# Annusha/LIReC

Measured on AMD Instinct MI355X. Metric: clips/sec fwd+bwd at 16 tracks×2048-d, higher is better.
Workload: dtype f32 in/out, bf16x3 split-precision MFMA, f32 accumulate

## Files before the change

include/lirec_hip.h:

```cpp
#ifndef LIREC_HIP_H
#define LIREC_HIP_H

#include <stdint.h>

#ifdef __cplusplus
extern "C" {
#endif

typedef void* lirec_stream_t;
typedef void* lirec_ctx_t;

#define LIREC_VERSION 124
#define LIREC_MAX_SEG 4

enum {
  LIREC_OK = 0,
  LIREC_EINVAL = 10001,
  LIREC_EWORKSPACE = 10002
};

enum { LIREC_SITE_H1_INTS = 0, LIREC_SITE_H1_CTX = 1, LIREC_SITE_E_INTS = 2,
       LIREC_SITE_E_CTX = 3, LIREC_SITE_GATE = 4,
       LIREC_SITE_TRACK_SAMPLE = 5 };

// ... 66 lines not shown
  const float* W2[LIREC_MAX_SEG];
  const float* H1;
  const float* dZ2; int64_t lddz2;
  float* dW1[LIREC_MAX_SEG]; float* db1[LIREC_MAX_SEG];
  float* dW2[LIREC_MAX_SEG]; float* db2[LIREC_MAX_SEG];
  void* workspace; int64_t workspace_bytes;
  const float* mask; const float* Hbar; const float* fscale;
  const int32_t* rowmap; const int32_t* cstart; const int32_t* count;
  const float* wts;
  int32_t in_off[LIREC_MAX_SEG], in_dim[LIREC_MAX_SEG], out_dim[LIREC_MAX_SEG];
  int32_t rows, nseg, J, parts;
  int32_t R, clamp_zero;
  lirec_rowsel sel;
  lirec_dropout drop;
  int32_t x_bf16, reserved2_;
  void* planes; int64_t planes_bytes;
  const void* hbits;
  const struct lirec_pieces_s* pieces;
  int32_t x_q32, reserved3_;
  const struct lirec_fused_adam_s* adam;
} lirec_embed_bwd_args;
typedef struct lirec_fused_adam_s {
  float* p; const float* g; float* m; float* v;
  void* wq; int64_t wq_first;
  int64_t n, n_params;
  int32_t step; float lr, beta1, beta2, eps, weight_decay, grad_scale;
  const int64_t* step_dev;
} lirec_fused_adam;
int lirec_embed_bwd(const lirec_embed_bwd_args* a, lirec_stream_t stream);
int lirec_embed_bwd2(const lirec_embed_bwd_args* a, const lirec_embed_bwd_args* b, lirec_stream_t stream);
typedef struct {
  const lirec_embed_bwd_args* heads[2];
  int32_t nh, out_bf16;
  const float* W1[2][LIREC_MAX_SEG];
  void* dX; int64_t ldx;
  int32_t n, rp1, D, reserved_;
} lirec_embed_dx_args;
int lirec_embed_dx(const lirec_embed_dx_args* a, lirec_stream_t stream);
int lirec_embed_dw1_indexed(const lirec_embed_bwd_args* const* heads, int32_t nh, const lirec_pieces* pieces,
                            float* const* P, float* const* S, lirec_stream_t stream);
typedef struct {
  const lirec_embed_bwd_args* heads[2];
  int32_t nh, reserved_;
  const float* S[2];
  const float* W1[2][LIREC_MAX_SEG];
  const lirec_pieces* pieces;
  float* dClip; int64_t ld_clip;
  float* dTrack; int64_t ld_track;
} lirec_embed_dx_indexed_args;
int lirec_embed_dx_indexed(const lirec_embed_dx_indexed_args* a, lirec_stream_t stream);
int64_t lirec_workspace_bytes(int32_t rows, int32_t nseg, int32_t J);
int64_t lirec_planes_bytes(int32_t rows, int32_t dsum, int32_t J, int32_t x_mode);

int lirec_pool_fwd(const float* Z2, int64_t ldz, const float* mask, int32_t n, int32_t R, int32_t W,
                   int32_t clamp_zero, float* Tn, int64_t ldtn, float* E, int64_t lde,
                   const lirec_dropout* drop, lirec_stream_t stream);
int lirec_pool_bwd(const float* dP, int64_t lddp, const float* mask, int32_t n, int32_t R, int32_t W,
                   int32_t clamp_zero, float* dZ2, int64_t lddz, lirec_stream_t stream);

int lirec_gate_fwd(const float* EE, int64_t ldee, const float* Wg, const float* bg, int32_t n, int32_t K,
                   int32_t N, float* G, int64_t ldg, const lirec_dropout* drop, lirec_stream_t stream);
int lirec_gate_bwd(const float* dZg, int64_t lddzg, const float* EE, int64_t ldee, const float* Wg,
                   int32_t n, int32_t K, int32_t N, int32_t split,
                   const float* Tn, int64_t ldtn, float* dWg, float* dbg, float* dEE, int64_t lddee,
                   int32_t acc_first, const lirec_dropout* drop, int32_t site_ctx, int32_t site_ints,
                   lirec_stream_t stream);
int lirec_gate_bwd_parts(const float* dZg, int64_t lddzg, const float* EE, int64_t ldee, const float* Wg,
                         int32_t n, int32_t K, int32_t N, int32_t split,
                         const float* Tn, int64_t ldtn, float* dWg, float* dbg, float* dEE, int64_t lddee,
                         int32_t acc_first, const lirec_dropout* drop, int32_t site_ctx, int32_t site_ints,
                         int32_t parts, lirec_stream_t stream);

int64_t lirec_gate_ws_bytes(int32_t n, int32_t K, int32_t N);
int lirec_gate_fwd_ws(const float* EE, int64_t ldee, const float* Wg, const float* bg, int32_t n, int32_t K,
                      int32_t N, float* G, int64_t ldg, const lirec_dropout* drop, void* ws, int64_t ws_bytes,
                      int32_t weights_staged, lirec_stream_t stream);
int lirec_gate_stage_weights(const float* Wg, int32_t n, int32_t K, int32_t N, void* ws, int64_t ws_bytes, lirec_stream_t stream);
int lirec_gate_bwd_ws(const float* dZg, int64_t lddzg, const float* EE, int64_t ldee, const float* Wg,
                      int32_t n, int32_t K, int32_t N, int32_t split,
                      const float* Tn, int64_t ldtn, float* dWg, float* dbg, float* dEE, int64_t lddee,
                      int32_t acc_first, const lirec_dropout* drop, int32_t site_ctx, int32_t site_ints,
                      int32_t parts, void* ws, int64_t ws_bytes, int32_t rows_staged, lirec_stream_t stream);

int lirec_linear_fwd(const float* A, int64_t lda, const float* W, const float* b, int32_t n, int32_t K,
                     int32_t N, float* Y, int64_t ldy, lirec_stream_t stream);
int lirec_linear_bwd(const float* dY, int64_t lddy, const float* A, int64_t lda, const float* W,
                     int32_t n, int32_t K, int32_t N, float* dW, float* db,
                     float* dA, int64_t ldda, int32_t mode, const float* act, int64_t ldact,
                     int32_t accumulate, const lirec_dropout* drop, lirec_stream_t stream);

typedef struct {
  const float* A; int64_t lda; const float* W; const float* b; float* Y; int64_t ldy;
  int32_t n, K, N, reserved_;
} lirec_linear_fwd_args;
int lirec_linear_fwd_group(const lirec_linear_fwd_args* v, int32_t count, lirec_stream_t stream);
typedef struct {
  const float* dY; int64_t lddy; const float* A; int64_t lda; const float* W;
  float* dW; float* db; float* dA; int64_t ldda; const float* act; int64_t ldact;
  int32_t n, K, N, mode, accumulate;
  int32_t parts;
  lirec_dropout drop;
} lirec_linear_bwd_args;
int lirec_linear_bwd_group(const lirec_linear_bwd_args* v, int32_t count, lirec_stream_t stream);

typedef struct {
  float* ints; int64_t ld_ints;
  const float* rels; int64_t ld_rels;
  const float* mem;
  const float* w;
  const int32_t* y;
  const int32_t* r;
  const int32_t* g;
  const int32_t* sel;
  float* d_ints; int64_t ld_dints;
  float* d_rels; int64_t ld_drels;
  float* loss;
  float* partial;
  int32_t* sel_out;
  int32_t B, T, C, NR;
  float margin, lymbda;
  int32_t max_neg, tr_correct, mask_inplace, rels_mean_valid;
  int32_t loader_types;
  int32_t sample;
  uint64_t sample_seed;
  const uint64_t* sample_seed_dev;
  float* probs_out;
  int32_t* arrive;
  float batch_divisor, rels_divisor;
  const float* divisors_dev;
  int32_t y_stride, reserved_;
} lirec_margin_loss_args;
int lirec_margin_loss(const lirec_margin_loss_args* a, lirec_stream_t stream);

int lirec_heads_loss_fwd_bwd(const lirec_linear_fwd_args* heads, const lirec_linear_bwd_args* back, int32_t n_heads,
                             const lirec_margin_loss_args* loss, lirec_stream_t stream);

int lirec_ce_loss(const float* ints, int64_t ld_ints, const float* rels, int64_t ld_rels,
                  const int32_t* y, const int32_t* r, const float* class_w,
                  int32_t B, int32_t C, int32_t NR, float* d_ints, int64_t ld_dints,
                  float* d_rels, int64_t ld_drels, float* loss, float* partial,
                  float den_ints, float den_rels, const float* dens_dev, lirec_stream_t stream);

int lirec_adam_step(float* p, const float* g, float* m, float* v, int64_t n, int32_t step,
                    float lr, float beta1, float beta2, float eps, float weight_decay,
                    float grad_scale, const int64_t* step_dev, lirec_stream_t stream);
int lirec_adam_step_counted(float* p, const float* g, float* m, float* v, int64_t n,
                            float lr, float beta1, float beta2, float eps, float weight_decay,
                            float grad_scale, int64_t* count_dev, int32_t* ticket, int32_t advance, lirec_stream_t stream);
int lirec_counter_add(int64_t* ctr, const int64_t* inc_host, int32_t n, lirec_stream_t stream);

typedef struct {
  const float* ints; int64_t ld_ints;
  const float* rels; int64_t ld_rels;
  const float* mem;
  const int32_t* y;
  const int32_t* r;
  const int32_t* g;
  const uint8_t* just_zeros;
  int64_t* counters;
  int32_t B, T, C, NR;
  int32_t loader_types, reserved_;
} lirec_eval_args;
int lirec_eval_max_tracks(const lirec_eval_args* a, lirec_stream_t stream);

int lirec_gather_features(const void* clip, int64_t ld_clip, const void* track, int64_t ld_track, int32_t table_f64,
                          const int32_t* index, int64_t rows, int32_t clip_dim, int32_t track_dim,
                          float* out, int64_t ld_out, lirec_stream_t stream);
int lirec_gather_features_bf16(const void* clip, int64_t ld_clip, const void* track, int64_t ld_track, int32_t table_f64,
                               const int32_t* index, int64_t rows, int32_t clip_dim, int32_t track_dim,
                               void* out, int64_t ld_out, lirec_stream_t stream);

int lirec_grid_pool(const float* grid, int32_t F, int32_t C, int32_t H, int32_t W, const int32_t* boxes,
                    const int32_t* estart, int32_t n_out, float* out, int64_t ld_out, lirec_stream_t stream);
int lirec_rows_max(const float* src, int64_t ld, const int32_t* idx, const int32_t* estart, int32_t n_out, int32_t dim,
                   float* out, int64_t ld_out, lirec_stream_t stream);

int lirec_cast_f64_f32(const double* src, float* dst, int64_t n, lirec_stream_t stream);
int lirec_dropout_mask(uint8_t* keep, int32_t rows, int32_t cols, const lirec_dropout* drop,
                       int32_t site, lirec_stream_t stream);
int lirec_version(void);
int lirec_abi_sizeof(int which);
int lirec_set_gemm_mode(int mode);
int lirec_get_gemm_mode(void);
int lirec_set_grad_overwrite(int on);
int lirec_grad_overwrite_conflicts(void);
const char* lirec_error_string(int code);
// ... 32 lines not shown
```

lirec_amd/_lib.py:

```python
from __future__ import annotations

import ctypes as C
import os

_HERE = os.path.dirname(os.path.abspath(__file__))
LIB_PATH = os.environ.get('LIREC_LIB_PATH') or os.path.join(_HERE, 'liblirec_hip.so')
MAX_SEG = 4
DEFAULT_GEMM_MODE = 2

SITE_H1_INTS, SITE_H1_CTX, SITE_E_INTS, SITE_E_CTX, SITE_GATE, SITE_TRACK_SAMPLE = 0, 1, 2, 3, 4, 5
ABI_VERSION = 124
LIREC_EINVAL = 10001

_vp, _i32, _i64, _f32 = C.c_void_p, C.c_int32, C.c_int64, C.c_float


class RowSel(C.Structure):
    _fields_ = [('group', _i32), ('group_stride', _i32), ('group_off', _i32)]


class Dropout(C.Structure):
    _fields_ = [('seed', C.c_uint64), ('p', _f32), ('site', _i32), ('site2', _i32), ('seed_dev', _vp)]


# ... 45 lines not shown
                ('margin', _f32), ('lymbda', _f32),
                ('max_neg', _i32), ('tr_correct', _i32), ('mask_inplace', _i32), ('rels_mean_valid', _i32),
                ('loader_types', _i32), ('sample', _i32),
                ('sample_seed', C.c_uint64), ('sample_seed_dev', _vp), ('probs_out', _vp), ('arrive', _vp),
                ('batch_divisor', _f32), ('rels_divisor', _f32), ('divisors_dev', _vp), ('y_stride', _i32), ('reserved_', _i32)]


class Pieces(C.Structure):
    _fields_ = [('clip', _vp), ('ld_clip', _i64), ('n_clip', _i32), ('track', _vp), ('ld_track', _i64), ('n_track', _i32),
                ('index', _vp), ('text_dim', _i32), ('visual_dim', _i32), ('track_dim', _i32),
                ('clip_q', _vp), ('track_q', _vp), ('clip_rows', _vp), ('track_rows', _vp)]


class EmbedDxIndexedArgs(C.Structure):
    _fields_ = [('heads', C.POINTER(EmbedBwdArgs) * 2), ('nh', _i32), ('reserved_', _i32), ('S', _vp * 2),
                ('W1', (_vp * MAX_SEG) * 2), ('pieces', C.POINTER(Pieces)),
                ('dClip', _vp), ('ld_clip', _i64), ('dTrack', _vp), ('ld_track', _i64)]


class LinearFwdArgs(C.Structure):
    _fields_ = [('A', _vp), ('lda', _i64), ('W', _vp), ('b', _vp), ('Y', _vp), ('ldy', _i64),
                ('n', _i32), ('K', _i32), ('N', _i32), ('reserved_', _i32)]


class LinearBwdArgs(C.Structure):
    _fields_ = [('dY', _vp), ('lddy', _i64), ('A', _vp), ('lda', _i64), ('W', _vp), ('dW', _vp), ('db', _vp), ('dA', _vp),
                ('ldda', _i64), ('act', _vp), ('ldact', _i64), ('n', _i32), ('K', _i32), ('N', _i32), ('mode', _i32),
                ('accumulate', _i32), ('parts', _i32), ('drop', Dropout)]


class EvalArgs(C.Structure):
    _fields_ = [('ints', _vp), ('ld_ints', _i64), ('rels', _vp), ('ld_rels', _i64), ('mem', _vp), ('y', _vp), ('r', _vp),
                ('g', _vp), ('just_zeros', _vp), ('counters', _vp), ('B', _i32), ('T', _i32), ('C', _i32), ('NR', _i32),
                ('loader_types', _i32), ('reserved_', _i32)]


class LirecError(RuntimeError):
    pass


_lib = None

_PROTOS = {
    'lirec_version': (_i32, []),
    'lirec_abi_sizeof': (_i32, [_i32]),
    'lirec_set_gemm_mode': (_i32, [_i32]),
    'lirec_get_gemm_mode': (_i32, []),
    'lirec_set_grad_overwrite': (_i32, [_i32]),
    'lirec_grad_overwrite_conflicts': (_i32, []),
    'lirec_ctx_create': (_i32, [C.POINTER(_vp)]),
    'lirec_ctx_destroy': (_i32, [_vp]),
    'lirec_ctx_set_current': (_i32, [_vp]),
    'lirec_ctx_get_current': (_vp, []),
    'lirec_debug_set': (_i32, [_i32, _i32]),
    'lirec_record_begin': (_i32, []),
    'lirec_record_mark': (_i32, []),
    'lirec_record_end': (_i32, [C.POINTER(_vp)]),
    'lirec_cmdlist_size': (_i32, [_vp]),
    'lirec_cmdlist_replay': (_i32, [_vp, _i32, _i32]),
    'lirec_cmdlist_replay_lagged': (_i32, [_vp, _i32, _i32, _i32, _i64]),
    'lirec_cmdlist_command': (_i32, [_vp, _i32, C.POINTER(_vp), C.POINTER(_i32)]),
    'lirec_cmdlist_destroy': (_i32, [_vp]),
    'lirec_stream_wait': (_i32, [_vp, _vp]),
    'lirec_stream_wait_many': (_i32, [C.POINTER(C.c_void_p), _i32, _vp]),
    'lirec_memset_zero': (_i32, [_vp, _i64, _vp]),
    'lirec_zero_count': (_i32, [_vp, _i64, _vp, C.POINTER(C.c_int64), _i32, _vp]),
    'lirec_error_string': (C.c_char_p, [_i32]),
    'lirec_workspace_bytes': (_i64, [_i32, _i32, _i32]),
    'lirec_planes_bytes': (_i64, [_i32, _i32, _i32, _i32]),
    'lirec_hbits_bytes': (_i64, [_i32, _i32]),
    'lirec_q32b_bytes': (_i64, [_i64, _i64]),
    'lirec_to_q32b': (_i32, [_vp, _i64, _i64, _i64, _vp, _vp]),
    'lirec_q16b_bytes': (_i64, [_i64, _i64]),
    'lirec_to_q16b': (_i32, [_vp, _i64, _i64, _i64, _vp, _vp]),
    'lirec_to_q16c': (_i32, [_vp, _i64, _i64, _i64, _vp, _vp]),
    'lirec_embed_fwd': (_i32, [C.POINTER(EmbedFwdArgs), _vp]),
    'lirec_embed_bwd': (_i32, [C.POINTER(EmbedBwdArgs), _vp]),
    'lirec_embed_fwd2': (_i32, [C.POINTER(EmbedFwdArgs), C.POINTER(EmbedFwdArgs), _vp]),
    'lirec_embed_dw1_indexed': (_i32, [C.POINTER(C.POINTER(EmbedBwdArgs)), _i32, C.POINTER(Pieces), C.POINTER(_vp), C.POINTER(_vp), _vp]),
    'lirec_embed_l1_indexed': (_i32, [C.POINTER(C.POINTER(EmbedFwdArgs)), _i32, C.POINTER(Pieces), C.POINTER(_vp), C.POINTER(_vp), _vp]),
    'lirec_embed_bwd2': (_i32, [C.POINTER(EmbedBwdArgs), C.POINTER(EmbedBwdArgs), _vp]),
    'lirec_embed_dx': (_i32, [C.POINTER(EmbedDxArgs), _vp]),
    'lirec_embed_dx_indexed': (_i32, [C.POINTER(EmbedDxIndexedArgs), _vp]),
    'lirec_linear_fwd_group': (_i32, [C.POINTER(LinearFwdArgs), _i32, _vp]),
    'lirec_linear_bwd_group': (_i32, [C.POINTER(LinearBwdArgs), _i32, _vp]),
    'lirec_compact_rows': (_i32, [_vp, _i32, _i32, _vp, _vp, _vp, _vp]),
    'lirec_compact_rows2': (_i32, [_vp, _i32, _i32, _i32, _vp, _vp, _vp, _vp, _vp]),
    'lirec_pool_fwd': (_i32, [_vp, _i64, _vp, _i32, _i32, _i32, _i32, _vp, _i64, _vp, _i64, C.POINTER(Dropout), _vp]),
    'lirec_pool_bwd': (_i32, [_vp, _i64, _vp, _i32, _i32, _i32, _i32, _vp, _i64, _vp]),
    'lirec_gate_fwd': (_i32, [_vp, _i64, _vp, _vp, _i32, _i32, _i32, _vp, _i64, C.POINTER(Dropout), _vp]),
    'lirec_gate_bwd': (_i32, [_vp, _i64, _vp, _i64, _vp, _i32, _i32, _i32, _i32, _vp, _i64, _vp, _vp, _vp, _i64,
                              _i32, C.POINTER(Dropout), _i32, _i32, _vp]),
    'lirec_gate_bwd_parts': (_i32, [_vp, _i64, _vp, _i64, _vp, _i32, _i32, _i32, _i32, _vp, _i64, _vp, _vp, _vp, _i64,
                                    _i32, C.POINTER(Dropout), _i32, _i32, _i32, _vp]),
    'lirec_gate_ws_bytes': (_i64, [_i32, _i32, _i32]),
    'lirec_gate_fwd_ws': (_i32, [_vp, _i64, _vp, _vp, _i32, _i32, _i32, _vp, _i64, C.POINTER(Dropout), _vp, _i64, _i32, _vp]),
    'lirec_gate_stage_weights': (_i32, [_vp, _i32, _i32, _i32, _vp, _i64, _vp]),
    'lirec_gate_bwd_ws': (_i32, [_vp, _i64, _vp, _i64, _vp, _i32, _i32, _i32, _i32, _vp, _i64, _vp, _vp, _vp, _i64,
                                 _i32, C.POINTER(Dropout), _i32, _i32, _i32, _vp, _i64, _i32, _vp]),
    'lirec_linear_fwd': (_i32, [_vp, _i64, _vp, _vp, _i32, _i32, _i32, _vp, _i64, _vp]),
    'lirec_linear_bwd': (_i32, [_vp, _i64, _vp, _i64, _vp, _i32, _i32, _i32, _vp, _vp, _vp, _i64, _i32, _vp, _i64,
                                _i32, C.POINTER(Dropout), _vp]),
    'lirec_margin_loss': (_i32, [C.POINTER(MarginLossArgs), _vp]),
    'lirec_heads_loss_fwd_bwd': (_i32, [C.POINTER(LinearFwdArgs), C.POINTER(LinearBwdArgs), _i32, C.POINTER(MarginLossArgs), _vp]),
    'lirec_ce_loss': (_i32, [_vp, _i64, _vp, _i64, _vp, _vp, _vp, _i32, _i32, _i32, _vp, _i64, _vp, _i64, _vp, _vp, _f32, _f32, _vp, _vp]),
    'lirec_adam_step': (_i32, [_vp, _vp, _vp, _vp, _i64, _i32, _f32, _f32, _f32, _f32, _f32, _f32, _vp, _vp]),
    'lirec_adam_step_counted': (_i32, [_vp, _vp, _vp, _vp, _i64, _f32, _f32, _f32, _f32, _f32, _f32, _vp, _vp, _i32, _vp]),
    'lirec_counter_add': (_i32, [_vp, C.POINTER(C.c_int64), _i32, _vp]),
    'lirec_eval_max_tracks': (_i32, [C.POINTER(EvalArgs), _vp]),
    'lirec_cast_f64_f32': (_i32, [_vp, _vp, _i64, _vp]),
    'lirec_grid_pool': (_i32, [_vp, _i32, _i32, _i32, _i32, _vp, _vp, _i32, _vp, _i64, _vp]),
    'lirec_rows_max': (_i32, [_vp, _i64, _vp, _vp, _i32, _i32, _vp, _i64, _vp]),
    'lirec_gather_features': (_i32, [_vp, _i64, _vp, _i64, _i32, _vp, _i64, _i32, _i32, _vp, _i64, _vp]),
    'lirec_gather_features_bf16': (_i32, [_vp, _i64, _vp, _i64, _i32, _vp, _i64, _i32, _i32, _vp, _i64, _vp]),
    'lirec_dropout_mask': (_i32, [_vp, _i32, _i32, C.POINTER(Dropout), _i32, _vp]),
    'lirec_set_scratch': (_i32, [_vp, _i64]),
    'lirec_profile_enable': (_i32, [_i32]),
    'lirec_profile_sites': (_i32, []),
    'lirec_profile_site_name': (C.c_char_p, [_i32]),
    'lirec_profile_read': (_i32, [_i32, C.POINTER(C.c_double), C.POINTER(_i64), C.POINTER(C.c_double),
                                  C.POINTER(C.c_double)]),
}

EXPORTS = tuple(_PROTOS)


def _bind_torch_hip_runtime():
    try:
        import torch
    except ImportError:
        return
    cand = os.path.join(os.path.dirname(torch.__file__), 'lib', 'libamdhip64.so')
    if os.path.exists(cand):
        C.CDLL(cand, mode=C.RTLD_GLOBAL)


def lib():
    global _lib
    if _lib is not None:
        return _lib
    if not os.path.exists(LIB_PATH):
        raise LirecError('HIP extension %s not found: build it first (python -c "import __graft_entry__ as g; '
                         'g.build()"). There is no fallback path.' % LIB_PATH)
    _bind_torch_hip_runtime()
    L = C.CDLL(LIB_PATH)
    for name, (res, args) in _PROTOS.items():
        fn = getattr(L, name)
        fn.restype, fn.argtypes = res, args
    for which, st in list(enumerate((EmbedFwdArgs, EmbedBwdArgs, MarginLossArgs, Dropout, RowSel))) + [(8, EmbedDxArgs),
                                                                                                      (9, EmbedDxIndexedArgs)]:
        if L.lirec_abi_sizeof(which) != C.sizeof(st):
            raise LirecError('ABI mismatch for %s: library %d bytes, binding %d bytes'
                             % (st.__name__, L.lirec_abi_sizeof(which), C.sizeof(st)))
    mode = os.environ.get('LIREC_GEMM_MODE', str(DEFAULT_GEMM_MODE))
    if L.lirec_set_gemm_mode(int(mode)) != 0:
        raise LirecError('LIREC_GEMM_MODE=%s is not a valid GEMM core (0 f32 MFMA, 1 naive, 2 bf16x3, 3 single-pass bf16)' % mode)
    _lib = L
    return L


def default_gemm_mode() -> int:
    return int(os.environ.get('LIREC_GEMM_MODE', DEFAULT_GEMM_MODE))


_calls = [0]

# ... 7 lines not shown
```

lirec_amd/csrc/gemm.hpp:

```cpp
#pragma once
#include <hip/hip_runtime.h>
#include <stdint.h>

namespace lirec {

typedef float f32x16 __attribute__((ext_vector_type(16)));
typedef float f32x4 __attribute__((ext_vector_type(4)));

enum { L_NT = 0, L_NN = 1, L_TN = 2 };
enum { EPI_STORE = 0, EPI_DROP_RELU = 1, EPI_TANH_DROP = 2, EPI_RELU_BWD = 3, EPI_TANH_BWD = 4 };

struct GemmProblem {
  const float* A; const float* B; float* C;
  const float* bias;
  const float* rowscale;
  const float* aux;
  float* aux_out;
  float* dbias;
  long lda, ldb, ldc, ldaux;
  int M, N, K;
  int gs, gstride, goff;
  unsigned gs_magic;
  int epi; float beta;
  int dbias_set;
  unsigned seed_lo, seed_hi, site, thresh; float drop_scale; int drop_col_off;
  const unsigned long long* seed_dev;
  int x_bf16;
  int tiles_n, tile_start;
  int ksplit, kchunk, tiles_mn;
  float* slab; float* dbias_slab;
  const int* rowmap; const int* dyn;
  const int* srow;
  const void* A_lo; const void* B_lo;
  unsigned char* xq_out; long ld_xq;
};

struct AdamFuse {
  float* p; const float* g; float* m; float* v;
  float step_size, bc2_sqrt, beta1, beta2, eps, wd, gscale, lr;
  const long long* step_dev;
  int wq16c;
};
__device__ __forceinline__ float adam1(const AdamFuse& ad, float step_size, float bc2_sqrt, long off, float g) {
#pragma clang fp contract(off)
  const float pp = ad.p[off];
  const float gg = g * ad.gscale + ad.wd * pp;
  const float mm = ad.m[off] + (1.f - ad.beta1) * (gg - ad.m[off]);
  const float vv = ad.v[off] * ad.beta2 + (1.f - ad.beta2) * gg * gg;
  ad.m[off] = mm; ad.v[off] = vv;
  const float pn = pp - step_size * (mm / (sqrtf(vv) / bc2_sqrt + ad.eps));
  ad.p[off] = pn;
  return pn;
}
__device__ __forceinline__ f32x4 adam4(const AdamFuse& ad, float step_size, float bc2_sqrt, long off, const f32x4 gv) {
#pragma clang fp contract(off)
  f32x4 pv = *reinterpret_cast<const f32x4*>(ad.p + off);
  f32x4 mv = *reinterpret_cast<const f32x4*>(ad.m + off);
  f32x4 vv = *reinterpret_cast<const f32x4*>(ad.v + off);
#pragma unroll
  for (int j = 0; j < 4; ++j) {
    const float gg = gv[j] * ad.gscale + ad.wd * pv[j];
    mv[j] = mv[j] + (1.f - ad.beta1) * (gg - mv[j]);
    vv[j] = vv[j] * ad.beta2 + (1.f - ad.beta2) * gg * gg;
    const float denom = sqrtf(vv[j]) / bc2_sqrt + ad.eps;
    pv[j] = pv[j] - step_size * (mv[j] / denom);
  }
  *reinterpret_cast<f32x4*>(ad.p + off) = pv;
  *reinterpret_cast<f32x4*>(ad.m + off) = mv;
  *reinterpret_cast<f32x4*>(ad.v + off) = vv;
  return pv;
}

#define LIREC_MAX_PROB 8
struct GemmGroup {
  int nprob; int total_tiles; int ablate; int row_tiles;
  const int* nt_bound;
  int nt_bound_val;
  int p3_tm, p3_tn, p3_xm;
  int nt_ct_major;
  int onepass;
  int tier_rows, row_tiles2, first2;
  int pgroup;
  int tm_fast;
  int tiles_per_split, resident_slots, dyn_is_k;
  int dyn_split;
  float slab_cost, reduce_cost;
  GemmProblem p[LIREC_MAX_PROB];
};
struct GemmMeta { int site; int tag; };

inline bool gemm_problem_is_vec(int layout, const GemmProblem& p) {
  const bool a_kc = layout != 2, b_kc = layout == 0;
  const uintptr_t ma = (p.x_bf16 && layout == 0) ? 7 : 15, mb = (p.x_bf16 && layout == 2) ? 7 : 15;
  const bool va = ((p.lda & 3) == 0) && ((reinterpret_cast<uintptr_t>(p.A) & ma) == 0) && (((a_kc ? p.K : p.M) & 3) == 0);
  const bool vb = ((p.ldb & 3) == 0) && ((reinterpret_cast<uintptr_t>(p.B) & mb) == 0) && (((b_kc ? p.K : p.N) & 3) == 0);
  return va && vb;
}

__device__ __forceinline__ void philox4(unsigned c0, unsigned c1, unsigned c2, unsigned c3,
                                        unsigned k0, unsigned k1, unsigned out[4]) {
#pragma unroll 2
  for (int i = 0; i < 10; ++i) {
    const unsigned long long p0 = (unsigned long long)0xD2511F53u * c0, p1 = (unsigned long long)0xCD9E8D57u * c2;
    const unsigned hi0 = (unsigned)(p0 >> 32), lo0 = (unsigned)p0;
    const unsigned hi1 = (unsigned)(p1 >> 32), lo1 = (unsigned)p1;
    const unsigned n0 = hi1 ^ c1 ^ k0, n2 = hi0 ^ c3 ^ k1;
    c0 = n0; c1 = lo1; c2 = n2; c3 = lo0;
    k0 += 0x9E3779B9u; k1 += 0xBB67AE85u;
  }
  out[0] = c0; out[1] = c1; out[2] = c2; out[3] = c3;
}

__device__ __forceinline__ void apply_seed_offset(unsigned& lo, unsigned& hi, const unsigned long long* seed_dev) {
  if (seed_dev) {
    const unsigned long long k = (((unsigned long long)hi << 32) | lo) + *seed_dev;
    lo = (unsigned)(k & 0xffffffffull); hi = (unsigned)(k >> 32);
  }
}

__device__ __forceinline__ bool epi_uses_dropout(const GemmProblem& p) {
  return p.thresh != 0u && (p.epi == EPI_DROP_RELU || p.epi == EPI_TANH_DROP || p.epi == EPI_TANH_BWD);
}

__device__ __forceinline__ float relu_f(float v) { return v > 0.f ? v : (v != v ? v : 0.f); }

__device__ __forceinline__ void epi_store(const GemmProblem& p, int row, int col, float acc, unsigned rnd) {
  float v = acc;
  if (p.bias) v += p.rowscale ? p.bias[col] * p.rowscale[row] : p.bias[col];
  float* cptr = p.C + (long)row * p.ldc + col;
  if (p.beta != 0.f) v += p.beta * (*cptr);
  switch (p.epi) {
    case EPI_DROP_RELU:
      v = relu_f(v);
      if (p.thresh) v = (rnd >= p.thresh) ? v * p.drop_scale : 0.f;
      break;
    case EPI_TANH_DROP: {
      const float t = tanhf(v);
      p.aux_out[(long)row * p.ldaux + col] = t;
      v = t;
      if (p.thresh) v = (rnd >= p.thresh) ? t * p.drop_scale : 0.f;
      break;
    }
    case EPI_RELU_BWD: {
      const float a = p.aux[(long)row * p.ldaux + col];
      v = (a > 0.f) ? v * p.drop_scale : 0.f;
      break;
    }
    case EPI_TANH_BWD: {
      const float t = p.aux[(long)row * p.ldaux + col];
      float f = 1.f - t * t;
      if (p.thresh) f = (rnd >= p.thresh) ? f * p.drop_scale : 0.f;
      v *= f;
      break;
    }
    default: break;
  }
  *cptr = v;
}

__device__ __forceinline__ int dyn_limit(const GemmProblem& p, int full) {
  if (!p.dyn) return full;
  const int d = *p.dyn;
  return d < full ? d : full;
}

__device__ __forceinline__ long sel_row(const GemmProblem& p, int n) {
  if (p.gs == 0) return n;
  const unsigned q = p.gs_magic ? __umulhi((unsigned)n, p.gs_magic) : (unsigned)n / (unsigned)p.gs;
  const unsigned r = (unsigned)n - q * (unsigned)p.gs;
  return (long)q * p.gstride + r + p.goff;
}
// ... 75 lines not shown
  TileCoord c;
  c.pi = 0;
  int tm;
  if (g.pgroup > 0) {
    const int G = g.pgroup, tier1 = g.tier_rows * g.row_tiles;
    const bool t2 = g.row_tiles2 > 0 && tile >= tier1;
    const int first = t2 ? g.first2 : 0, np = t2 ? g.nprob - g.first2 : g.nprob;
    const int rt = t2 ? g.row_tiles2 : g.row_tiles;
    const int rows = t2 ? g.p[first].tiles_mn / g.p[first].tiles_n - g.tier_rows : g.tier_rows;
    const int t = t2 ? tile - tier1 : tile;
    const int tn_each = g.p[first].tiles_n;
    const int blk = t / (G * rt);
    const int within = t - blk * G * rt;
    const int per = min(G, rows - blk * G) * tn_each;
    const int q = within / per, r2 = within - q * per;
    const int rot = (blk * np) / 8 + (t2 ? 1 : 0);
    c.pi = first + (q + rot) % np;
    const int pr = r2 / tn_each;
    c.tn = r2 - pr * tn_each;
    c.split = 0;
    tm = (t2 ? g.tier_rows : 0) + blk * G + pr;
  } else if (g.row_tiles > 0) {
    const int tier1 = g.tier_rows * g.row_tiles;
    if (g.row_tiles2 > 0 && tile >= tier1) {
      const int t2 = tile - tier1;
      const int row2 = t2 / g.row_tiles2;
      const int rem = t2 - row2 * g.row_tiles2 + g.p[g.first2].tile_start;
      c.pi = g.first2;
#pragma unroll
      for (int i = 1; i < LIREC_MAX_PROB; ++i)
        if (i > g.first2 && i < g.nprob && rem >= g.p[i].tile_start) c.pi = i;
      c.tn = rem - g.p[c.pi].tile_start;
      c.split = 0;
      tm = g.tier_rows + row2;
    } else {
      const int tiles_m = g.p[0].tiles_mn / g.p[0].tiles_n;
      int row, rem;
      if (g.tm_fast) {
        const int per_split = tiles_m * g.row_tiles;
        c.split = tile / per_split;
        const int r = tile - c.split * per_split;
        rem = r / tiles_m;
        tm = r - rem * tiles_m;
      } else {
        row = tile / g.row_tiles;
        rem = tile - row * g.row_tiles;
        c.split = row / tiles_m;
        tm = row - c.split * tiles_m;
      }
#pragma unroll
      for (int i = 1; i < LIREC_MAX_PROB; ++i)
        if (i < g.nprob && rem >= g.p[i].tile_start) c.pi = i;
      c.tn = rem - g.p[c.pi].tile_start;
    }
  } else {
#pragma unroll
    for (int i = 1; i < LIREC_MAX_PROB; ++i)
      if (i < g.nprob && tile >= g.p[i].tile_start) c.pi = i;
    int t = tile - g.p[c.pi].tile_start;
    c.split = t / g.p[c.pi].tiles_mn;
    t -= c.split * g.p[c.pi].tiles_mn;
    tm = t / g.p[c.pi].tiles_n;
    c.tn = t - tm * g.p[c.pi].tiles_n;
  }
  const GemmProblem& p = g.p[c.pi];
  c.m0 = tm * BM; c.n0 = c.tn * BN;
  int K = p.K, kchunk = p.kchunk;
  c.M = p.M;
  if (p.dyn) {
    if (dyn_is_k) {
      K = dyn_limit(p, p.K);
      const int ks = effective_ksplit(g, p, K);
      kchunk = ((K + ks - 1) / ks + 31) / 32 * 32;
      if (c.split >= ks) c.M = 0;
    } else {
      c.M = dyn_limit(p, p.M);
    }
  }
  c.k_begin = min(K, c.split * kchunk);
  c.k_end = min(K, c.k_begin + kchunk);
  return c;
}

template <int WM, int WN, int EPI>
__device__ __forceinline__ void gemm_epilogue_kind(const GemmProblem& p, const f32x16 (&acc)[WM][WN], int m0, int n0,
                                                   int wm0, int wn0, int lane, int M, bool have_rid = false, int rid_lane = 0) {
  constexpr bool USES_RND = (EPI == EPI_DROP_RELU || EPI == EPI_TANH_DROP || EPI == EPI_TANH_BWD);
  constexpr bool USES_AUX = (EPI == EPI_RELU_BWD || EPI == EPI_TANH_BWD);
  const int l31 = lane & 31, lh = lane >> 5;
  const int N = p.N;
  const bool drop = USES_RND && p.thresh != 0u;
  unsigned key_lo = p.seed_lo, key_hi = p.seed_hi;
  if (drop) apply_seed_offset(key_lo, key_hi, p.seed_dev);
  const bool mapped = drop && (p.rowmap != nullptr);
  const bool has_beta = p.beta != 0.f, has_rs = p.bias != nullptr && p.rowscale != nullptr;
  float bias_j[WN];
#pragma unroll
  for (int j = 0; j < WN; ++j) {
    const int col = n0 + wn0 + 32 * j + l31;
    bias_j[j] = (p.bias != nullptr && col < N) ? p.bias[col] : 0.f;
  }
  constexpr bool PRE_AUX = USES_AUX && (WM * WN <= 2);
#pragma unroll
  for (int i = 0; i < WM; ++i) {
#pragma unroll
    for (int j = 0; j < WN; ++j) {
      const int col = n0 + wn0 + 32 * j + l31;
      const bool colok = col < N;
      float axp[PRE_AUX ? 16 : 1];
      if constexpr (PRE_AUX) {
#pragma unroll
        for (int q = 0; q < 4; ++q)
#pragma unroll
          for (int jj = 0; jj < 4; ++jj) {
            const int row = m0 + wm0 + 32 * i + 8 * q + 4 * lh + jj;
            const bool okk = colok && row < M;
            axp[4 * q + jj] = p.aux[(long)(okk ? row : m0) * p.ldaux + (okk ? col : n0)];
          }
      }
#pragma unroll
      for (int q = 0; q < 4; ++q) {
        const int row4 = m0 + wm0 + 32 * i + 8 * q + 4 * lh;
        if (row4 >= M) continue;
        bool ok[4];
        float* cptr[4];
        float old[4] = {0.f, 0.f, 0.f, 0.f}, ax[4] = {0.f, 0.f, 0.f, 0.f}, rs[4] = {1.f, 1.f, 1.f, 1.f};
#pragma unroll
        for (int jj = 0; jj < 4; ++jj) {
          ok[jj] = colok && (row4 + jj < M);
          const int r = ok[jj] ? row4 + jj : m0, c = ok[jj] ? col : n0;
          cptr[jj] = p.C + (long)r * p.ldc + c;
          if (has_beta) old[jj] = *cptr[jj];
          if constexpr (PRE_AUX) ax[jj] = axp[4 * q + jj];
          else if constexpr (USES_AUX) ax[jj] = p.aux[(long)r * p.ldaux + c];
          if (has_rs) rs[jj] = p.rowscale[r];
        }
        unsigned w[4] = {0u, 0u, 0u, 0u};
        if (drop) {
          if (!mapped) {
            philox4((unsigned)(p.drop_col_off + col), (unsigned)(row4 >> 2), p.site, 0u, key_lo, key_hi, w);
          } else {
            unsigned rid[4], rnd[4];
#pragma unroll
            for (int jj = 0; jj < 4; ++jj) {
              if (have_rid) rid[jj] = (unsigned)__shfl(rid_lane, 32 * i + 8 * q + 4 * lh + jj, 64);
              else rid[jj] = (unsigned)p.rowmap[row4 + jj < M ? row4 + jj : M - 1];
            }
            unsigned blk = rid[0] >> 2;
            philox4((unsigned)(p.drop_col_off + col), blk, p.site, 0u, key_lo, key_hi, rnd);
#pragma unroll
            for (int jj = 0; jj < 4; ++jj) {
              if ((rid[jj] >> 2) != blk) {
                blk = rid[jj] >> 2;
                philox4((unsigned)(p.drop_col_off + col), blk, p.site, 0u, key_lo, key_hi, rnd);
              }
              const unsigned k = rid[jj] & 3u;
              w[jj] = k == 0u ? rnd[0] : (k == 1u ? rnd[1] : (k == 2u ? rnd[2] : rnd[3]));
            }
          }
        }
#pragma unroll
        for (int jj = 0; jj < 4; ++jj) {
          float v = acc[i][j][4 * q + jj] + bias_j[j] * rs[jj] + p.beta * old[jj];
          const bool keep = !drop || w[jj] >= p.thresh;
          if constexpr (EPI == EPI_DROP_RELU) {
            v = relu_f(v);
            v = keep ? v * p.drop_scale : 0.f;
          } else if constexpr (EPI == EPI_TANH_DROP) {
            const float t = tanhf(v);
            if (ok[jj]) p.aux_out[(long)(row4 + jj) * p.ldaux + col] = t;
            v = keep ? t * p.drop_scale : 0.f;
          } else if constexpr (EPI == EPI_RELU_BWD) {
            v = (ax[jj] > 0.f) ? v * p.drop_scale : 0.f;
          } else if constexpr (EPI == EPI_TANH_BWD) {
            const float f = 1.f - ax[jj] * ax[jj];
            v *= keep ? f * p.drop_scale : 0.f;
          }
          if (ok[jj]) *cptr[jj] = v;
        }
        __asm__ volatile("" ::: "memory");
      }
    }
  }
}

__host__ __device__ constexpr bool epi_allowed(int layout, int epi) {
  return epi == EPI_STORE || (layout == L_NT && (epi == EPI_DROP_RELU || epi == EPI_TANH_DROP)) ||
         (layout == L_NN && (epi == EPI_RELU_BWD || epi == EPI_TANH_BWD));
}

template <int WM, int WN, int LAYOUT>
__device__ __forceinline__ void gemm_epilogue(const GemmProblem& p, const f32x16 (&acc)[WM][WN], int m0, int n0,
                                              int wm0, int wn0, int lane, int split, int M_eff, bool have_rid = false, int rid_lane = 0) {
  const int l31 = lane & 31, lh = lane >> 5;
  const int M = M_eff, N = p.N;
  if (p.ksplit > 1) {
    float* slab = p.slab + (long)split * p.M * N;
#pragma unroll
    for (int i = 0; i < WM; ++i)
#pragma unroll
      for (int j = 0; j < WN; ++j) {
        const int col = n0 + wn0 + 32 * j + l31;
#pragma unroll
        for (int r = 0; r < 16; ++r) {
          const int row = m0 + wm0 + 32 * i + (r & 3) + 8 * (r >> 2) + 4 * lh;
          if (row < M && col < N) slab[(long)row * N + col] = acc[i][j][r];
        }
      }
    return;
  }
  if constexpr (LAYOUT == L_NT) {
    if (p.epi == EPI_DROP_RELU) gemm_epilogue_kind<WM, WN, EPI_DROP_RELU>(p, acc, m0, n0, wm0, wn0, lane, M, have_rid, rid_lane);
    else if (p.epi == EPI_TANH_DROP) gemm_epilogue_kind<WM, WN, EPI_TANH_DROP>(p, acc, m0, n0, wm0, wn0, lane, M);
    else gemm_epilogue_kind<WM, WN, EPI_STORE>(p, acc, m0, n0, wm0, wn0, lane, M);
  } else if constexpr (LAYOUT == L_NN) {
    if (p.epi == EPI_RELU_BWD) gemm_epilogue_kind<WM, WN, EPI_RELU_BWD>(p, acc, m0, n0, wm0, wn0, lane, M);
    else if (p.epi == EPI_TANH_BWD) gemm_epilogue_kind<WM, WN, EPI_TANH_BWD>(p, acc, m0, n0, wm0, wn0, lane, M);
    else gemm_epilogue_kind<WM, WN, EPI_STORE>(p, acc, m0, n0, wm0, wn0, lane, M);
  } else {
    gemm_epilogue_kind<WM, WN, EPI_STORE>(p, acc, m0, n0, wm0, wn0, lane, M);
  }
}

static __global__ __launch_bounds__(256) void splitk_reduce_kernel(const GemmGroup g) {
  for (int pi = 0; pi < g.nprob; ++pi) {
    const GemmProblem& p = g.p[pi];
    if (p.ksplit <= 1) continue;
    const int ks = (p.dyn && g.dyn_is_k) ? effective_ksplit(g, p, dyn_limit(p, p.K)) : p.ksplit;
    const long mn = (long)p.M * p.N;
    const long gtid = (long)blockIdx.x * blockDim.x + threadIdx.x, gsz = (long)gridDim.x * blockDim.x;
    const bool vec4 = (p.N % 4 == 0) && (p.ldc % 4 == 0) && ((((size_t)p.C) | ((size_t)p.slab)) % 16 == 0);
    if (p.epi != EPI_STORE) {
      const bool drop = p.thresh != 0u && (p.epi == EPI_DROP_RELU || p.epi == EPI_TANH_DROP || p.epi == EPI_TANH_BWD);
      unsigned key_lo = p.seed_lo, key_hi = p.seed_hi;
      if (drop) apply_seed_offset(key_lo, key_hi, p.seed_dev);
      const long groups = (long)((p.M + 3) >> 2) * p.N;
      for (long e = gtid; e < groups; e += gsz) {
        const int r4 = (int)(e / p.N), col = (int)(e - (long)r4 * p.N), row0 = r4 << 2;
        float v[4] = {0.f, 0.f, 0.f, 0.f};
        for (int sidx = 0; sidx < ks; ++sidx) {
          const float* sl = p.slab + (long)sidx * mn + (long)row0 * p.N + col;
#pragma unroll
          for (int jj = 0; jj < 4; ++jj) if (row0 + jj < p.M) v[jj] += sl[(long)jj * p.N];
        }
        unsigned w[4] = {0u, 0u, 0u, 0u};
        if (drop) philox4((unsigned)(p.drop_col_off + col), (unsigned)r4, p.site, 0u, key_lo, key_hi, w);
        const float b = p.bias ? p.bias[col] : 0.f;
#pragma unroll
        for (int jj = 0; jj < 4; ++jj) {
          const int row = row0 + jj;
          if (row >= p.M) continue;
          float* c = p.C + (long)row * p.ldc + col;
          float x = v[jj] + b * ((p.bias && p.rowscale) ? p.rowscale[row] : 1.f) + (p.beta != 0.f ? p.beta * (*c) : 0.f);
          const bool keep = !drop || w[jj] >= p.thresh;
          if (p.epi == EPI_DROP_RELU) {
            x = relu_f(x);
            x = keep ? x * p.drop_scale : 0.f;
          } else if (p.epi == EPI_TANH_DROP) {
            const float t = tanhf(x);
            p.aux_out[(long)row * p.ldaux + col] = t;
            x = keep ? t * p.drop_scale : 0.f;
          } else if (p.epi == EPI_RELU_BWD) {
            x = (p.aux[(long)row * p.ldaux + col] > 0.f) ? x * p.drop_scale : 0.f;
          } else if (p.epi == EPI_TANH_BWD) {
            const float t = p.aux[(long)row * p.ldaux + col];
            const float f = 1.f - t * t;
            x *= keep ? f * p.drop_scale : 0.f;
          }
          *c = x;
        }
      }
    } else if (vec4) {
      const long mn4 = mn >> 2;
      const int n4 = p.N >> 2;
      for (long e = gtid; e < mn4; e += gsz) {
        const int row = (int)(e / n4), col = (int)(e - (long)row * n4) * 4;
        const f32x4* src = (const f32x4*)p.slab + e;
        f32x4* c = (f32x4*)(p.C + (long)row * p.ldc + col);
        f32x4 o = {0.f, 0.f, 0.f, 0.f};
        if (p.beta != 0.f) o = *c;
        f32x4 v = src[0];
        int s = 1;
        for (; s + 3 < ks; s += 4) {
          const f32x4 t0 = src[(long)s * mn4], t1 = src[(long)(s + 1) * mn4], t2 = src[(long)(s + 2) * mn4], t3 = src[(long)(s + 3) * mn4];
#pragma unroll
          for (int j = 0; j < 4; ++j) { v[j] += t0[j]; v[j] += t1[j]; v[j] += t2[j]; v[j] += t3[j]; }
        }
        for (; s < ks; ++s) { const f32x4 t = src[(long)s * mn4]; v[0] += t[0]; v[1] += t[1]; v[2] += t[2]; v[3] += t[3]; }
        if (p.bias) {
          const float rs = p.rowscale ? p.rowscale[row] : 1.f;
#pragma unroll
          for (int j = 0; j < 4; ++j) v[j] += p.bias[col + j] * rs;
        }
        if (p.beta != 0.f) { v[0] += p.beta * o[0]; v[1] += p.beta * o[1]; v[2] += p.beta * o[2]; v[3] += p.beta * o[3]; }
        *c = v;
      }
    } else {
      for (long e = gtid; e < mn; e += gsz) {
        const int row = (int)(e / p.N), col = (int)(e - (long)row * p.N);
// ... 296 lines not shown
```

lirec_amd/csrc/gemm_bf16x3.hpp:

```cpp
#pragma once
#include <type_traits>
#include "gemm.hpp"

namespace lirec {

typedef __bf16 bf16x8 __attribute__((ext_vector_type(8)));
typedef __bf16 bf16x4 __attribute__((ext_vector_type(4)));
typedef short s16x4 __attribute__((ext_vector_type(4)));
typedef short s16x8 __attribute__((ext_vector_type(8)));

typedef float f32x2 __attribute__((ext_vector_type(2)));
typedef __bf16 bf16x2 __attribute__((ext_vector_type(2)));
__device__ __forceinline__ void split4(const f32x4 v, uint2& hi, uint2& lo) {
  const f32x2 v01 = {v[0], v[1]}, v23 = {v[2], v[3]};
  const bf16x2 h01 = __builtin_convertvector(v01, bf16x2), h23 = __builtin_convertvector(v23, bf16x2);
  const unsigned w01 = __builtin_bit_cast(unsigned, h01), w23 = __builtin_bit_cast(unsigned, h23);
  const f32x2 f01 = {__builtin_bit_cast(float, w01 << 16), __builtin_bit_cast(float, w01 & 0xffff0000u)};
  const f32x2 f23 = {__builtin_bit_cast(float, w23 << 16), __builtin_bit_cast(float, w23 & 0xffff0000u)};
  const f32x2 r01 = v01 - f01, r23 = v23 - f23;
  const bf16x2 l01 = __builtin_convertvector(r01, bf16x2), l23 = __builtin_convertvector(r23, bf16x2);
  hi = make_uint2(w01, w23);
  lo = make_uint2(__builtin_bit_cast(unsigned, l01), __builtin_bit_cast(unsigned, l23));
}

__device__ __forceinline__ uint2 hi4(const f32x4 v) {
  const f32x2 v01 = {v[0], v[1]}, v23 = {v[2], v[3]};
  const bf16x2 h01 = __builtin_convertvector(v01, bf16x2), h23 = __builtin_convertvector(v23, bf16x2);
  return make_uint2(__builtin_bit_cast(unsigned, h01), __builtin_bit_cast(unsigned, h23));
}

__device__ __forceinline__ void p2_store_q32b(unsigned char* dst, long row, int c8, int cblocks, const f32x4 a, const f32x4 b) {
  uint2 h0, l0, h1, l1;
  split4(a, h0, l0);
  split4(b, h1, l1);
  unsigned char* blk = dst + (((row >> 5) * cblocks + (c8 >> 2)) * 32 + (row & 31)) * 128 + (c8 & 3) * 16;
  *reinterpret_cast<uint4*>(blk) = make_uint4(h0.x, h0.y, h1.x, h1.y);
  *reinterpret_cast<uint4*>(blk + 64) = make_uint4(l0.x, l0.y, l1.x, l1.y);
}

__device__ __forceinline__ void p2_store_q16b(unsigned char* dst, long row, int c8, int cblocks, const f32x4 a, const f32x4 b) {
  const uint2 h0 = hi4(a), h1 = hi4(b);
  unsigned char* blk = dst + (((row >> 5) * cblocks + (c8 >> 2)) * 32 + (row & 31)) * 64 + (c8 & 3) * 16;
  *reinterpret_cast<uint4*>(blk) = make_uint4(h0.x, h0.y, h1.x, h1.y);
}

__device__ __forceinline__ long p2_q16c_off(long row, int c8, int cblocks64) {
  return (((row >> 5) * cblocks64 + (c8 >> 3)) * 32 + (row & 31)) * 128 + (c8 & 7) * 16;
}
__device__ __forceinline__ void p2_store_q16c(unsigned char* dst, long row, int c8, int cblocks64, const f32x4 a, const f32x4 b) {
  const uint2 h0 = hi4(a), h1 = hi4(b);
  *reinterpret_cast<uint4*>(dst + p2_q16c_off(row, c8, cblocks64)) = make_uint4(h0.x, h0.y, h1.x, h1.y);
}

__device__ __forceinline__ s16x4 lds_tr16(const unsigned char* p) {
  return __builtin_amdgcn_ds_read_tr16_b64_v4i16(
      (s16x4 __attribute__((address_space(3)))*)(reinterpret_cast<const s16x4*>(p)));
}

template <bool KC, int EXT>
struct OperandTile {
  static constexpr int BK = 32;
  static constexpr int PITCH = KC ? (BK * 2) : (EXT * 2 + 64);
  static constexpr int BYTES = KC ? EXT * PITCH : BK * PITCH;
  static constexpr int NCH = EXT / 32;
};

template <int CFG> struct TileCfg;
template <> struct TileCfg<0> { static constexpr int WAVES_M = 2, WAVES_N = 2, WM = 1, WN = 1; };
template <> struct TileCfg<1> { static constexpr int WAVES_M = 2, WAVES_N = 2, WM = 2, WN = 2; };
template <> struct TileCfg<2> { static constexpr int WAVES_M = 2, WAVES_N = 4, WM = 4, WN = 2; };
template <> struct TileCfg<3> { static constexpr int WAVES_M = 4, WAVES_N = 2, WM = 1, WN = 2; };
template <> struct TileCfg<4> { static constexpr int WAVES_M = 4, WAVES_N = 2, WM = 2, WN = 2; };

template <int LAYOUT, int CFG, int TAG, bool VEC, bool XB = false>
__global__ __launch_bounds__(64 * TileCfg<CFG>::WAVES_M * TileCfg<CFG>::WAVES_N, (CFG == 3 ? 4 : 2)) void gemm_bf16x3_kernel(const GemmGroup g) {
  constexpr int WAVES_M = TileCfg<CFG>::WAVES_M, WAVES_N = TileCfg<CFG>::WAVES_N;
  constexpr int WM = TileCfg<CFG>::WM, WN = TileCfg<CFG>::WN;
  constexpr int NTHR = 64 * WAVES_M * WAVES_N;
  constexpr int BM = 32 * WM * WAVES_M, BN = 32 * WN * WAVES_N, BK = 32;
  constexpr bool A_KC = (LAYOUT != L_TN);
  constexpr bool B_KC = (LAYOUT == L_NT);
  static_assert(!XB || (VEC && LAYOUT != L_NN), "bf16 X: dword-aligned staging, forward or weight-gradient layout");
  constexpr bool AXB = XB && LAYOUT == L_NT, BXB = XB && LAYOUT == L_TN;
  using TA = OperandTile<A_KC, BM>;
  using TB = OperandTile<B_KC, BN>;
  constexpr int BUF = 2 * (TA::BYTES + TB::BYTES);
  constexpr int RP = NTHR / 8;
  constexpr int QA = BM / 4, QB = BN / 4;
  constexpr int KSA = NTHR / QA, KSB = NTHR / QB;
  constexpr int CA = A_KC ? BM / RP : BK / KSA;
  constexpr int CB = B_KC ? BN / RP : BK / KSB;
  __shared__ __attribute__((aligned(16))) unsigned char smem[2 * BUF];

  const int tid = threadIdx.x, lane = tid & 63, wave = tid >> 6;
  const int ltile = launch_tile(g);
  if (ltile < 0) return;
  const TileCoord tc = decode_tile<BM, BN>(g, ltile, LAYOUT == L_TN);
  const GemmProblem& p = g.p[tc.pi];
  const int m0 = tc.m0, n0 = tc.n0;
  const int M = tc.M, N = p.N, K = tc.k_end, kb = tc.k_begin;
  if (m0 >= M) return;
  const bool interior = (m0 + BM <= M) && (n0 + BN <= N) && (((K - kb) & (BK - 1)) == 0);

  const float* a_rowptr[A_KC ? CA : 1];
  const float* b_rowptr[B_KC ? CB : 1];
  bool a_rowok[A_KC ? CA : 1], b_rowok[B_KC ? CB : 1];
// ... 173 lines not shown
    } else {
      const unsigned char* q = img + b_frag + 64 * j + 16 * s * TB::PITCH;
      const s16x4 x = lds_tr16(q), y = lds_tr16(q + 4 * TB::PITCH);
      const s16x8 v = {x[0], x[1], x[2], x[3], y[0], y[1], y[2], y[3]};
      return *reinterpret_cast<const bf16x8*>(&v);
    }
  };

  constexpr int NGROUP = 2 * WM * WN;
  auto ktile = [&](int buf, int k0_next, int k0_next2, auto store_tag, auto load_tag, auto edge_tag, auto one_tag) __attribute__((always_inline)) {
    constexpr bool STORE_NEXT = decltype(store_tag)::value, LOAD_NEXT2 = decltype(load_tag)::value;
    constexpr bool ONE = decltype(one_tag)::value;
    const unsigned char* a_hi = smem + buf * BUF;
    const unsigned char* a_lo = a_hi + TA::BYTES;
    const unsigned char* b_hi = a_lo + TA::BYTES;
    const unsigned char* b_lo = b_hi + TB::BYTES;
#pragma unroll
    for (int s = 0; s < 2; ++s) {
      bf16x8 ah[WM], al[WM], bh[WN], bl[WN];
#pragma unroll
      for (int i = 0; i < WM; ++i) { ah[i] = frag_a(a_hi, i, s); if constexpr (!AXB && !ONE) al[i] = frag_a(a_lo, i, s); }
#pragma unroll
      for (int j = 0; j < WN; ++j) { bh[j] = frag_b(b_hi, j, s); if constexpr (!BXB && !ONE) bl[j] = frag_b(b_lo, j, s); }
#pragma unroll
      for (int i = 0; i < WM; ++i)
#pragma unroll
        for (int j = 0; j < WN; ++j) {
          if constexpr (!AXB && !ONE) acc[i][j] = __builtin_amdgcn_mfma_f32_32x32x16_bf16(al[i], bh[j], acc[i][j], 0, 0, 0);
          if constexpr (!BXB && !ONE) acc[i][j] = __builtin_amdgcn_mfma_f32_32x32x16_bf16(ah[i], bl[j], acc[i][j], 0, 0, 0);
          acc[i][j] = __builtin_amdgcn_mfma_f32_32x32x16_bf16(ah[i], bh[j], acc[i][j], 0, 0, 0);
          const int grp = (s * WM + i) * WN + j;
#pragma unroll
          for (int c = grp * NCHUNK / NGROUP; c < (grp + 1) * NCHUNK / NGROUP; ++c) {
            if constexpr (STORE_NEXT) store_chunk(buf ^ 1, k0_next, c, edge_tag, one_tag);
            if constexpr (LOAD_NEXT2) load_chunk(k0_next2, c, edge_tag);
          }
        }
    }
  };

  auto mainloop = [&](auto edge_tag, auto one_tag) __attribute__((always_inline)) {
    const int nk = (K - kb + BK - 1) / BK;
    if (nk <= 0) return;
    if constexpr (LAYOUT == L_TN) {
      if (tn_mapped) {
#pragma unroll
        for (int i = 0; i < CB; ++i) {
          const int k = kb + b_kr + KSB * i;
          b_nextrow[i] = p.rowmap[k < K ? k : (K > 0 ? K - 1 : 0)];
        }
      }
    }
#pragma unroll
    for (int c = 0; c < NCHUNK; ++c) load_chunk(kb, c, edge_tag);
#pragma unroll
    for (int c = 0; c < NCHUNK; ++c) {
      store_chunk(0, kb, c, edge_tag, one_tag);
      if (nk > 1) load_chunk(kb + BK, c, edge_tag);
    }
    __syncthreads();
    int kt = 0;
    for (; kt + 2 < nk; ++kt) {
      ktile(kt & 1, kb + (kt + 1) * BK, kb + (kt + 2) * BK, std::true_type{}, std::true_type{}, edge_tag, one_tag);
      __syncthreads();
    }
    if (kt + 1 < nk) {
      ktile(kt & 1, kb + (kt + 1) * BK, 0, std::true_type{}, std::false_type{}, edge_tag, one_tag);
      __syncthreads();
      ++kt;
    }
    ktile(kt & 1, 0, 0, std::false_type{}, std::false_type{}, edge_tag, one_tag);
    __syncthreads();
  };
  constexpr bool ONE_OK = !(LAYOUT == L_TN && TAG == 0 && (CFG == 1 || CFG == 2 || CFG == 4));
  bool one = false;
  if constexpr (ONE_OK) one = g.onepass != 0;
  if (g.ablate & 4) {  }
  else if (one) {
    if constexpr (ONE_OK) { if (interior) mainloop(std::false_type{}, std::true_type{}); else mainloop(std::true_type{}, std::true_type{}); }
  }
  else if (interior) mainloop(std::false_type{}, std::false_type{});
  else mainloop(std::true_type{}, std::false_type{});

  gemm_epilogue<WM, WN, LAYOUT>(p, acc, m0, n0, wm0, wn0, lane, tc.split, M);

  if constexpr (LAYOUT == L_TN) {
    if (do_dbias) {
      float* red = reinterpret_cast<float*>(smem);
      __syncthreads();
#pragma unroll
      for (int c = 0; c < 4; ++c) red[tid * 4 + c] = dbias_acc[c];
      __syncthreads();
      if (tid < QA) {
        float v[4] = {0.f, 0.f, 0.f, 0.f};
        for (int r = 0; r < KSA; ++r)
#pragma unroll
          for (int c = 0; c < 4; ++c) v[c] += red[(tid + QA * r) * 4 + c];
#pragma unroll
        for (int c = 0; c < 4; ++c) {
          const int m = m0 + 4 * tid + c;
          if (m < M) {
            if (p.ksplit > 1) p.dbias_slab[(long)tc.split * p.M + m] = v[c];
            else p.dbias[m] = p.dbias_set ? v[c] : p.dbias[m] + v[c];
          }
        }
      }
    }
  }
}

}
```

lirec_amd/csrc/lirec_hip.hip:

```cpp
#include <hip/hip_runtime.h>
#include <math.h>
#include <stdlib.h>
#include <string.h>
#include <new>

#include "lirec_hip.h"
#include "gemm.hpp"
#include "gemm_launch.hpp"
#include "kernels.hpp"
#include "gemm_dx.hpp"

using namespace lirec;

thread_local lirec::CmdList* lirec::t_rec = nullptr;
bool lirec::g_dry = false;
struct lirec_cmdlist { lirec::CmdList list; };

struct lirec_ctx {
  int gemm_mode = 0;
  int ablate = 0;
  int force_cfg = -1;
  float* scratch = nullptr;
  long scratch_floats = 0;
};
// ... 168 lines not shown
      g.row_tiles = off;
      g.tier_rows = tiles_m(0);
      if (two) { g.first2 = first2; g.row_tiles2 = off - g.p[first2].tile_start; }
      bool eq = unsplit && !(g_ablate & 256);
      for (int i = 1; i < g.nprob; ++i) eq = eq && g.p[i].tiles_n == g.p[0].tiles_n;
      const int tn = g.p[0].tiles_n;
      if (eq && tn <= 16 && 32 % tn == 0 && g.tier_rows >= 32 / tn) g.pgroup = 32 / tn;
    }
  }
  {
    bool ok = g.p[0].ksplit > 1 && g.p[0].dyn != nullptr && (g.nprob == 1 || (g.row_tiles > 0 && g.row_tiles2 == 0));
    for (int i = 1; ok && i < g.nprob; ++i) ok = g.p[i].ksplit == g.p[0].ksplit && g.p[i].dyn == g.p[0].dyn && g.p[i].K == g.p[0].K;
    g.dyn_split = ok ? 1 : 0;
  }
  g.tm_fast = (g.dyn_is_k && g.row_tiles > 0 && g.row_tiles2 == 0 && !(g_ablate & 512)) ? 1 : 0;
  return start;
}
static void launch_splitk_reduce(const GemmGroup& g, hipStream_t s) {
  ReducePlan rp;
  memset(&rp, 0, sizeof(rp));
  bool plain = !(g_ablate & (64 | 128 | 4096));
  int blocks = 0;
  for (int i = 0; i < g.nprob; ++i) {
    const GemmProblem& p = g.p[i];
    if (p.ksplit <= 1) continue;
    plain = plain && p.epi == EPI_STORE && !(p.dyn && g.dyn_split && (g_ablate & 64));
    const bool vec4 = (p.N % 4 == 0) && (p.ldc % 4 == 0) && ((((size_t)p.C) | ((size_t)p.slab)) % 16 == 0);
    long items = vec4 ? ((long)p.M * p.N) >> 2 : (long)p.M * p.N;
    if (p.dbias && p.dbias_slab && items < p.M) items = p.M;
    rp.prob[rp.n] = i;
    rp.start[rp.n++] = blocks;
    blocks += (int)((items + 255) / 256);
  }
  rp.start[rp.n] = blocks;
  if (plain && rp.n > 0 && blocks > 0) lirec::launch(splitk_reduce_flat_kernel, dim3((unsigned)blocks), dim3(256), 0, s, g, rp);
  else lirec::launch(splitk_reduce_kernel, dim3(1024), dim3(256), 0, s, g);
}

static int plan_tiles(GemmGroup& g, int bm, int bn, int ksplit_want, bool& any_split) {
  int ks[LIREC_MAX_PROB];
  for (int i = 0; i < LIREC_MAX_PROB; ++i) ks[i] = ksplit_want;
  return plan_tiles_v(g, bm, bn, ks, any_split);
}

template <int LAYOUT>
static int launch_layout_(GemmGroup& g, GemmMeta meta, hipStream_t s);

template <int LAYOUT>
static int launch_layout(GemmGroup& g, GemmMeta meta, hipStream_t s) {
  if (g.nprob <= 0) return LIREC_OK;
  double flops = 0.0;
  for (int i = 0; i < g.nprob; ++i) flops += 2.0 * g.p[i].M * (double)g.p[i].N * g.p[i].K;
  const int pi = prof_start(meta.site, s);
  const int rc = launch_layout_<LAYOUT>(g, meta, s);
  prof_stop(pi, s, flops, 0.0);
  return rc;
}

template <int LAYOUT>
static int launch_layout_(GemmGroup& g, GemmMeta meta, hipStream_t s) {
  for (int i = 0; i < g.nprob; ++i)
    if (!epi_allowed(LAYOUT, g.p[i].epi)) return LIREC_EINVAL;
  if (g_gemm_mode == 1) {
    for (int i = 0; i < g.nprob; ++i) {
      GemmProblem& p = g.p[i];
      p.ksplit = 1;
      if (p.M <= 0 || p.N <= 0) continue;
      dim3 grid((p.N + 15) / 16, (p.M + 15) / 16);
      if (LAYOUT == L_NT) launch_naive_L0(grid, s, p);
      else if (LAYOUT == L_NN) launch_naive_L1(grid, s, p);
      else launch_naive_L2(grid, s, p);
      LIREC_CHECK_LAUNCH();
    }
    return LIREC_OK;
  }
  long t256 = 0, t128 = 0, t64 = 0, mn_total = 0;
  bool splittable = g_scratch != nullptr && !t_no_split, wide = true, wide256 = true, deep = true, any_epi = false;
  for (int i = 0; i < g.nprob; ++i) {
    const GemmProblem& p = g.p[i];
    t256 += (long)((p.M + 255) / 256) * ((p.N + 255) / 256);
    t128 += (long)((p.M + 127) / 128) * ((p.N + 127) / 128);
    t64 += (long)((p.M + 63) / 64) * ((p.N + 63) / 64);
    mn_total += (long)p.M * p.N + (p.dbias ? p.M : 0);
    splittable = splittable && p.K >= 512 && (p.epi == EPI_STORE || (p.rowmap == nullptr && p.dyn == nullptr && p.K >= 2048 &&
                                                                     (g_ablate & 128)));
    any_epi = any_epi || p.epi != EPI_STORE;
    wide = wide && p.M >= 96 && p.N >= 96;
    wide256 = wide256 && p.M >= 192 && p.N >= 192;
    deep = deep && p.K >= 4096;
  }
  static const int cfg_bm[5] = {64, 128, 256, 128, 256}, cfg_bn[5] = {64, 128, 256, 128, 128};
  const bool huge = g_bf_core && wide256 && splittable && deep && !any_epi;
  const bool big = !huge && (t128 >= (LAYOUT == L_NN ? 160 : 384) || (splittable && wide));
  int cfg = huge ? 2 : (big ? 3 : 0);
  if (!g_bf_core && LAYOUT == L_NN && !splittable && cfg != 0 && t128 < 256) {
    long kmin = 1L << 40;
    for (int i = 0; i < g.nprob; ++i) kmin = g.p[i].K < kmin ? g.p[i].K : kmin;
    if (kmin >= 2048) cfg = 0;
  }
  if (g_force_cfg >= 0 && g_force_cfg < 5) cfg = g_force_cfg;
  if (cfg == 2 && LAYOUT != L_TN) cfg = 3;
  if (!g_bf_core) cfg = (cfg == 0) ? 0 : 1;
  const int bm = cfg_bm[cfg], bn = cfg_bn[cfg];
  long t0 = 0;
  for (int i = 0; i < g.nprob; ++i) t0 += (long)((g.p[i].M + bm - 1) / bm) * ((g.p[i].N + bn - 1) / bn);
  const long fill = (bm * bn > 128 * 128) ? 256 : 512;
  int ksplit_want = 1;
  if (splittable && cfg == 0) {
    if (t0 < fill) ksplit_want = (int)((3 * fill / 2 + t0 - 1) / t0);
  } else if (splittable) {
    long kmax = 0, kmin = 1L << 40;
    for (int i = 0; i < g.nprob; ++i) { kmax = g.p[i].K > kmax ? g.p[i].K : kmax; kmin = g.p[i].K < kmin ? g.p[i].K : kmin; }
    const double tk_alone = !g_bf_core ? 3.4 : ((bm * bn == 256 * 256) ? 2.8 : (bm * bn == 256 * 128 ? 1.6 : 1.0));
    const double tk_shared = !g_bf_core ? 4.0 : ((bm * bn == 128 * 128) ? 1.2 : tk_alone);
    double best = 1e30;
    for (int ks = 1; ks <= 32; ++ks) {
      if (ks > 1 && kmin / ks < 256) break;
      if (ks > 1 && (long)ks * mn_total > g_scratch_floats) break;
      const long blocks = t0 * ks;
      const long slots = ((any_epi || !g_bf_core) && bm * bn == 128 * 128) ? 512 : 256;
      const double rounds = (double)((blocks + slots - 1) / slots);
      const double nk = (double)((kmax + ks - 1) / ks + 31) / 32;
      double cost = rounds * nk * (blocks > 256 ? tk_shared : tk_alone);
      if (ks > 1) cost += 6.0 + (double)(ks + 1) * (double)mn_total * 4.0 / 4.0e6;
      if (cost < best) { best = cost; ksplit_want = ks; }
    }
  }
  if (ksplit_want > 1 && mn_total > 0) {
    const long fit = g_scratch_floats / mn_total;
    if (fit < ksplit_want) ksplit_want = fit > 1 ? (int)fit : 1;
  }
  bool any_split = false;
  const int start = plan_tiles(g, bm, bn, ksplit_want, any_split);
  if (start == 0) return LIREC_OK;
  constexpr int T1 = (LAYOUT == L_NT) ? 1 : (LAYOUT == L_TN ? 2 : 0);
  bool vec = true;
  for (int i = 0; i < g.nprob; ++i) vec = vec && gemm_problem_is_vec(LAYOUT, g.p[i]);
  bool mapped = (LAYOUT == L_TN);
  for (int i = 0; i < g.nprob; ++i) mapped = mapped && g.p[i].rowmap != nullptr;
  bool unmapped = true;
  for (int i = 0; i < g.nprob; ++i) unmapped = unmapped && g.p[i].rowmap == nullptr;
  int variant = !vec ? GV_SCALAR : ((T1 != 0 && meta.tag == T1) ? GV_TAGGED : GV_VEC);
  if (LAYOUT == L_TN && variant == GV_TAGGED) variant = mapped ? GV_MAPPED : (unmapped ? GV_TAGGED : GV_VEC);
  bool xb_all = true, xb_any = false;
  for (int i = 0; i < g.nprob; ++i) { xb_all = xb_all && g.p[i].x_bf16; xb_any = xb_any || g.p[i].x_bf16; }
  if (xb_any) {
    if (!xb_all || !g_bf_core || LAYOUT == L_NN || (variant != GV_TAGGED && variant != GV_MAPPED)) return LIREC_EINVAL;
    variant = (variant == GV_MAPPED) ? GV_MAPPED_XB : GV_TAGGED_XB;
  }
  const dim3 grid(start);
  typedef void (*bf_fn)(int, dim3, hipStream_t, const GemmGroup&);
  typedef void (*f32_fn)(bool, int, dim3, hipStream_t, const GemmGroup&);
  static const bf_fn bf_table[3][5] = {
      {launch_bf_L0_C0, launch_bf_L0_C1, launch_bf_L0_C3, launch_bf_L0_C3, launch_bf_L0_C4},
      {launch_bf_L1_C0, launch_bf_L1_C1, launch_bf_L1_C3, launch_bf_L1_C3, launch_bf_L1_C4},
      {launch_bf_L2_C0, launch_bf_L2_C1, launch_bf_L2_C2, launch_bf_L2_C3, launch_bf_L2_C4}};
  static const f32_fn f32_table[3] = {launch_f32_L0, launch_f32_L1, launch_f32_L2};
  g.onepass = (g_gemm_mode == 3) && (meta.site == PS_EMBED_L1_FWD || meta.site == PS_EMBED_DW1 || meta.site == PS_GATE_FWD ||
                                     meta.site == PS_GATE_DW || meta.site == PS_GATE_DEE);
  if (g_bf_core) bf_table[LAYOUT][cfg](variant, grid, s, g);
  else f32_table[LAYOUT](cfg != 0, variant, grid, s, g);
  if (any_split) {
    LIREC_CHECK_LAUNCH();
    launch_splitk_reduce(g, s);
  }
  LIREC_CHECK_LAUNCH();
  return LIREC_OK;
// ... 726 lines not shown
    int given = 0;
    for (int i = 0; i < hs[h]->nseg; ++i) given += hs[h]->W1q[i] != nullptr;
    if (given != 0 && given != hs[h]->nseg) return LIREC_EINVAL;
    for (int i = 0; planes && i < hs[h]->nseg; ++i) {
      if (given) {
        if ((reinterpret_cast<uintptr_t>(hs[h]->W1q[i]) & 255) != 0) return LIREC_EINVAL;
        L[h].wq[i] = reinterpret_cast<unsigned char*>(const_cast<void*>(hs[h]->W1q[i]));
      } else {
        planes = splitq_add(q, hs[h]->W1[i], L[h].wq[i], hs[h]->J, hs[h]->in_dim[i]);
      }
    }
  }
  for (int h = 0; !planes && h < nh; ++h)
    if (hs[h]->W1q[0]) return LIREC_EINVAL;
  if (planes) {
    GemmGroup m;
    m.nprob = 0;
    for (int h = 0; !rc && h < nh; ++h) {
      for (int i = 0; i < hs[h]->nseg; ++i) {
        GemmProblem p = g1[h].p[i];
        if (hs[h]->drop.p > 0.f) { p.aux = reinterpret_cast<const float*>(L[h].keep); p.ldaux = (long)hs[h]->nseg * hs[h]->J; }
        if (L[h].gather) {
          gather_operand(hs[h], L[h], i, p.A, p.lda, p.srow);
        } else {
          p.A = reinterpret_cast<const float*>(L[h].xq + 4096L * ((hs[h]->in_off[i] - L[h].c0) / 32));
          p.lda = L[h].dsum;
        }
        p.B = reinterpret_cast<const float*>(L[h].wq[i]); p.ldb = hs[h]->in_dim[i];
        if (g_gemm_mode == 3) {
          p.K >>= 1; p.lda >>= 1; p.ldb >>= 1;
        }
        p.gs = 0; p.gs_magic = 0; p.x_bf16 = 0;
        m.p[m.nprob++] = p;
      }
    }
    {
      StageFused f;
      memset(&f, 0, sizeof(f));
      const int first = (nh == 2 && hs[1]->rows > hs[0]->rows) ? 1 : 0;
      double bytes = 0.0;
      for (int k = 0; k < nh && stage_mode != 2; ++k) {
        const int h = (k == 0) ? first : 1 - first;
        stage_head_fill(f.h[k], hs[h], L[h]);
        if (L[h].staged16) bytes += 4.0 * (double)hs[h]->rows * L[h].dsum;
        else if (!L[h].gather) bytes += 8.0 * (double)hs[h]->rows * L[h].dsum;
      }
      f.nh = stage_mode == 2 ? 0 : nh;
      if (stage_mode != 1) {
        f.w = q;
        long wb = (q.first[q.nseg] + 255) / 256;
        f.w_blocks = (int)(wb > 2048 ? 2048 : wb);
        bytes += 64.0 * (double)q.first[q.nseg];
      }
      f.part.grid = p2_grid(); f.part.out = stage_mode == 2 ? nullptr : L[0].nt_bound;
      for (int i = 0; i < m.nprob; ++i)
        if (m.p[i].M > 0 && m.p[i].N > 0) {
          const int k = f.part.n++;
          f.part.ks[k] = m.p[i].K >> 5; f.part.rows[k] = m.p[i].M; f.part.dyn[k] = m.p[i].dyn; f.part.nrep = m.p[i].N / 256;
        }
      long grid = f.w_blocks + 1;
      for (int k = 0; k < f.nh; ++k) grid += f.h[k].blocks;
      if (f.nh > 0 || f.w_blocks > 0 || f.part.out) {
        if ((g_ablate & 262144) && stage_mode == 1) lirec::launch(spin_kernel, dim3(1), dim3(64), 0, s, 200000LL);
        const int pi = prof_start(PS_STAGE, s);
        lirec::launch(stage_fused_kernel, dim3((unsigned)grid), dim3(256), 0, s, f);
        prof_stop(pi, s, 0.0, bytes);
        LIREC_CHECK_LAUNCH();
      }
    }
    if (stage_mode == 1) return rc;
    if (!rc) rc = launch_p2<L_NT>(m, s, PS_EMBED_L1_FWD, L[0].nt_bound, 0, L[0].gather, nullptr, L[0].gather ? gather_planes(hs, nh) : 2);
  } else {
    GemmGroup m;
    if (nh == 2 && merge_groups(g1[0], g1[1], m)) {
      rc = launch_gemm(L_NT, m, s, PS_EMBED_L1_FWD, 1);
    } else {
      for (int h = 0; !rc && h < nh; ++h) rc = launch_gemm(L_NT, g1[h], s, PS_EMBED_L1_FWD, 1);
    }
  }
  for (int h = 0; !rc && h < nh; ++h) rc = embed_fwd_pool_only(hs[h], s);
  return rc;
}

int lirec_embed_fwd(const lirec_embed_fwd_args* a, lirec_stream_t stream) {
  GemmGroup g1, g2;
  int rc = embed_fwd_build(a, g1, g2);
  if (rc) return rc;
  if (a->rows == 0) return LIREC_OK;
  if (a->parts < 0 || a->parts > 4) return LIREC_EINVAL;
  hipStream_t s = (hipStream_t)stream;
  if (a->parts == 4) return embed_fwd_layer1_heads(&a, &g1, 1, s, 1);
  if (a->parts == 3) rc = embed_fwd_pool_only(a, s);
  else if (a->parts != 2) rc = embed_fwd_layer1_heads(&a, &g1, 1, s, a->rows_staged ? 2 : 0);
  if (rc || a->parts == 1) return rc;
  return launch_gemm(L_NT, g2, s, PS_EMBED_L2_FWD);
}

int lirec_embed_fwd2(const lirec_embed_fwd_args* a, const lirec_embed_fwd_args* b, lirec_stream_t stream) {
  GemmGroup g1[2], a2, b2, m2;
  int rc = embed_fwd_build(a, g1[0], a2);
  if (rc) return rc;
  rc = embed_fwd_build(b, g1[1], b2);
  if (rc) return rc;
  if (a->rows == 0 || b->rows == 0) {
    rc = lirec_embed_fwd(a, stream);
    return rc ? rc : lirec_embed_fwd(b, stream);
  }
  hipStream_t s = (hipStream_t)stream;
  if (a->parts < 0 || a->parts > 4 || b->parts != a->parts || (a->rows_staged != 0) != (b->rows_staged != 0)) return LIREC_EINVAL;
  const lirec_embed_fwd_args* hs[2] = {a, b};
  if (a->parts == 4) return embed_fwd_layer1_heads(hs, g1, 2, s, 1);
  if (a->parts == 3) { rc = embed_fwd_pool_only(a, s); if (!rc) rc = embed_fwd_pool_only(b, s); }
  else if (a->parts != 2) rc = embed_fwd_layer1_heads(hs, g1, 2, s, a->rows_staged ? 2 : 0);
  if (rc || a->parts == 1) return rc;
  if (merge_groups(a2, b2, m2)) return launch_gemm(L_NT, m2, s, PS_EMBED_L2_FWD);
  rc = launch_gemm(L_NT, a2, s, PS_EMBED_L2_FWD);
  return rc ? rc : launch_gemm(L_NT, b2, s, PS_EMBED_L2_FWD);
}

int lirec_embed_l1_indexed(const lirec_embed_fwd_args* const* heads, int32_t nh, const lirec_pieces* pc,
                           float* const* zclip, float* const* ztrk, lirec_stream_t stream) {
  if (!heads || !pc || !zclip || !ztrk || nh < 1 || nh > 2 || !pc->clip || !pc->track || !pc->index || pc->n_clip < 1 || pc->n_track < 1)
    return LIREC_EINVAL;
  hipStream_t s = (hipStream_t)stream;
  GemmGroup g;
  memset(&g, 0, sizeof(g));
  for (int h = 0; h < nh; ++h) {
    const lirec_embed_fwd_args* a = heads[h];
    if (!a || !a->H1 || a->nseg != 4 || a->J < 256 || (a->J & 255) || a->rows < 0 || !zclip[h] || !ztrk[h] || a->x_bf16) return LIREC_EINVAL;
    if (a->in_dim[0] != pc->text_dim || a->in_dim[1] != pc->visual_dim || a->in_dim[2] != pc->track_dim || a->in_dim[3] != pc->track_dim)
      return LIREC_EINVAL;
    const int J = a->J;
    for (int i = 0; i < 4; ++i) {
      if (!a->W1[i] || !a->b1[i]) return LIREC_EINVAL;
      GemmProblem p = make_problem();
      if (i < 2) { p.A = pc->clip + (i == 0 ? 0 : pc->text_dim); p.lda = pc->ld_clip; p.M = pc->n_clip; p.C = zclip[h] + (long)i * J; }
      else { p.A = pc->track; p.lda = pc->ld_track; p.M = pc->n_track; p.C = ztrk[h] + (long)(i - 2) * J; }
      p.B = a->W1[i]; p.ldb = a->in_dim[i];
      p.ldc = 2L * J; p.N = J; p.K = a->in_dim[i];
      p.epi = EPI_STORE;
      g.p[g.nprob++] = p;
    }
  }
  t_no_split = true;
  int rc = launch_gemm(L_NT, g, s, PS_EMBED_L1_FWD);
  t_no_split = false;
  for (int h = 0; !rc && h < nh; ++h) {
    const lirec_embed_fwd_args* a = heads[h];
    if (a->rows == 0) continue;
    const bool compact = a->rowmap != nullptr;
    GatherActArgs ga;
    memset(&ga, 0, sizeof(ga));
    ga.zclip = zclip[h]; ga.ld_zclip = 2L * a->J; ga.ztrk = ztrk[h]; ga.ld_ztrk = 2L * a->J;
    ga.index = pc->index;
    ga.gs = a->sel.group; ga.gstride = a->sel.group_stride; ga.goff = a->sel.group_off; ga.gs_magic = row_magic(ga.gs, a->rows);
    for (int i = 0; i < 4; ++i) ga.b1[i] = a->b1[i];
    ga.rowmap = compact ? a->rowmap : nullptr; ga.count = compact ? a->count : nullptr;
    ga.H1 = a->H1; ga.ldh = 4L * a->J; ga.rows = a->rows; ga.J = a->J;
    const float p = a->drop.p;
    ga.seed_lo = (unsigned)(a->drop.seed & 0xffffffffull); ga.seed_hi = (unsigned)(a->drop.seed >> 32);
    ga.seed_dev = (const unsigned long long*)a->drop.seed_dev; ga.site = (unsigned)a->drop.site;
    ga.thresh = drop_thresh(p); ga.scale = (p > 0.f) ? (float)(1.0 / (1.0 - (double)p)) : 1.f;
    int gy = (a->rows + 3) / 4;
    if (gy > 256) gy = 256;
    const int pi = prof_start(PS_STAGE, s);
    lirec::launch(gather_act_kernel, dim3((unsigned)(4 * a->J / 256), (unsigned)gy), dim3(256), 0, s, ga);
    prof_stop(pi, s, 0.0, 4.0 * (double)a->rows * 4 * a->J);
    LIREC_CHECK_LAUNCH();
  }
  return rc;
}

static int embed_bwd_build(const lirec_embed_bwd_args* a, GemmGroup& gw2, GemmGroup& gdz, GemmGroup& gw1) {
  if (!a || (!a->X && a->parts != 1 && a->parts != 3 && a->parts != 5 && !a->planes) || (!a->H1 && !a->hbits) || !a->dZ2 || a->nseg < 1 || a->nseg > LIREC_MAX_SEG || a->J < 1 || a->rows < 0)
    return LIREC_EINVAL;
  const bool pooled = a->mask != nullptr || a->rowmap != nullptr;
  if (a->hbits && !pooled) return LIREC_EINVAL;
  if (pooled && (!a->Hbar || !a->fscale || a->R < 1 || a->rows % a->R != 0)) return LIREC_EINVAL;
  const bool compact = pooled && a->rowmap != nullptr;
  if ((a->rowmap || a->cstart || a->count) && !(a->rowmap && a->cstart && a->count && (a->mask || a->wts))) return LIREC_EINVAL;
  if (a->wts && !compact) return LIREC_EINVAL;
  const int J = a->J, nseg = a->nseg;
  const int n2 = pooled ? a->rows / a->R : a->rows;
  if (!a->workspace || a->workspace_bytes < lirec_workspace_bytes(a->rows + (pooled ? n2 : 0), nseg, J)) return LIREC_EWORKSPACE;
  float* dZ1 = (float*)a->workspace;
  float* dHbar = dZ1 + (long)((a->rows + 31) / 32 * 32) * nseg * J;
  const long ldh = (long)nseg * J;
  const float scale = (a->drop.p > 0.f) ? (float)(1.0 / (1.0 - (double)a->drop.p)) : 1.f;
  gw2.nprob = gdz.nprob = gw1.nprob = nseg;
  int ooff = 0;
  for (int i = 0; i < nseg; ++i) {
    if (!a->W2[i] || !a->dW1[i] || !a->dW2[i] || !a->db1[i] || !a->db2[i]) return LIREC_EINVAL;
    GemmProblem p = make_problem();
    p.A = a->dZ2 + ooff; p.lda = a->lddz2;
    p.B = (pooled ? a->Hbar : a->H1) + (long)i * J; p.ldb = ldh;
    p.C = a->dW2[i]; p.ldc = J;
    p.M = a->out_dim[i]; p.N = J; p.K = n2;
    p.beta = grad_beta(); p.dbias_set = g_grad_overwrite; p.dbias = a->db2[i];
    p.rowscale = pooled ? a->fscale : nullptr;
    gw2.p[i] = p;
// ... 446 lines not shown

int lirec_pool_fwd(const float* Z2, int64_t ldz, const float* mask, int32_t n, int32_t R, int32_t W,
                   int32_t clamp_zero, float* Tn, int64_t ldtn, float* E, int64_t lde,
                   const lirec_dropout* drop, lirec_stream_t stream) {
  if (!Z2 || !mask || !Tn || !E || n < 0 || R < 1 || W < 1) return LIREC_EINVAL;
  if (n == 0) return LIREC_OK;
  return launch_pool(Z2, (long)ldz, mask, n, R, W, clamp_zero, Tn, (long)ldtn, E, (long)lde, drop, 0, nullptr,
                     (hipStream_t)stream);
}

int lirec_pool_bwd(const float* dP, int64_t lddp, const float* mask, int32_t n, int32_t R, int32_t W,
                   int32_t clamp_zero, float* dZ2, int64_t lddz, lirec_stream_t stream) {
  if (!dP || !mask || !dZ2 || n < 0 || R < 1 || W < 1) return LIREC_EINVAL;
  if (n == 0) return LIREC_OK;
  const int pi = prof_start(PS_POOL_BWD, (hipStream_t)stream);
  lirec::launch(pool_bwd_kernel, dim3(n), dim3(256), 0, (hipStream_t)stream, dP, (long)lddp, mask, R, W,
                     clamp_zero, dZ2, (long)lddz);
  prof_stop(pi, (hipStream_t)stream, 0.0, 4.0 * n * ((double)R * W + R + W));
  LIREC_CHECK_LAUNCH();
  return LIREC_OK;
}

int lirec_gate_fwd(const float* EE, int64_t ldee, const float* Wg, const float* bg, int32_t n, int32_t K,
                   int32_t N, float* G, int64_t ldg, const lirec_dropout* drop, lirec_stream_t stream) {
  if (!EE || !Wg || !G || n < 0 || K < 1 || N < 1) return LIREC_EINVAL;
  GemmGroup g; g.nprob = 1;
  GemmProblem p = make_problem();
  p.A = EE; p.lda = ldee; p.B = Wg; p.ldb = K; p.bias = bg; p.C = G; p.ldc = ldg;
  p.M = n; p.N = N; p.K = K; p.epi = EPI_DROP_RELU;
  set_dropout(p, drop, drop ? drop->site : LIREC_SITE_GATE, 0);
  g.p[0] = p;
  return launch_gemm(L_NT, g, (hipStream_t)stream, PS_GATE_FWD);
}

int lirec_gate_bwd(const float* dZg, int64_t lddzg, const float* EE, int64_t ldee, const float* Wg,
                   int32_t n, int32_t K, int32_t N, int32_t split,
                   const float* Tn, int64_t ldtn, float* dWg, float* dbg, float* dEE, int64_t lddee,
                   int32_t acc_first, const lirec_dropout* drop, int32_t site_ctx, int32_t site_ints,
                   lirec_stream_t stream) {
  return lirec_gate_bwd_parts(dZg, lddzg, EE, ldee, Wg, n, K, N, split, Tn, ldtn, dWg, dbg, dEE, lddee, acc_first, drop, site_ctx,
                              site_ints, 0, stream);
}

int lirec_gate_bwd_parts(const float* dZg, int64_t lddzg, const float* EE, int64_t ldee, const float* Wg,
                         int32_t n, int32_t K, int32_t N, int32_t split,
                         const float* Tn, int64_t ldtn, float* dWg, float* dbg, float* dEE, int64_t lddee,
                         int32_t acc_first, const lirec_dropout* drop, int32_t site_ctx, int32_t site_ints,
                         int32_t parts, lirec_stream_t stream) {
  if (!dZg || !EE || !Wg || !Tn || !dWg || !dbg || !dEE || n < 0 || K < 1 || N < 1 || split < 0 || split > K || parts < 0 || parts > 2)
    return LIREC_EINVAL;
  hipStream_t s = (hipStream_t)stream;
  int rc = LIREC_OK;
  if (parts != 2) {
    GemmGroup gw; gw.nprob = 1;
    GemmProblem w = make_problem();
    w.A = dZg; w.lda = lddzg; w.B = EE; w.ldb = ldee; w.C = dWg; w.ldc = K;
    w.M = N; w.N = K; w.K = n; w.beta = grad_beta(); w.dbias_set = g_grad_overwrite; w.dbias = dbg;
    gw.p[0] = w;
    rc = launch_gemm(L_TN, gw, s, PS_GATE_DW);
  }
  if (rc || parts == 1) return rc;
  GemmGroup gd; gd.nprob = 2;
  for (int h = 0; h < 2; ++h) {
    const int c0 = h == 0 ? 0 : split, nc = h == 0 ? split : K - split;
    GemmProblem p = make_problem();
    p.A = dZg; p.lda = lddzg;
    p.B = Wg + c0; p.ldb = K;
    p.C = dEE + c0; p.ldc = lddee;
    p.M = n; p.N = nc; p.K = N;
    p.epi = EPI_TANH_BWD; p.aux = Tn + c0; p.ldaux = ldtn;
    p.beta = (h == 0 && acc_first) ? 1.f : 0.f;
    set_dropout(p, drop, h == 0 ? site_ctx : site_ints, 0);
    gd.p[h] = p;
  }
  return launch_gemm(L_NN, gd, s, PS_GATE_DEE);
}

static bool gate_p3_ok(int n, int K, int N, int split);
static bool gate_q32_ok(int n, int K, int N, int64_t ldee, const void* ws, int64_t ws_bytes) {
  return (g_gemm_mode == 2 || (g_gemm_mode == 3 && gate_p3_ok(n, K, N, K / 2))) && !(g_ablate & 8) && ws != nullptr &&
         (reinterpret_cast<uintptr_t>(ws) & 255) == 0 && n >= 32 && (n & 31) == 0 &&
         (K & 255) == 0 && (N & 255) == 0 && ldee == K && ws_bytes >= lirec_gate_ws_bytes(n, K, N);
}
struct GateWs { unsigned char* wq; unsigned char* eq; unsigned char* zq; unsigned char* wqT; unsigned char* eqT; unsigned char* zqT; };
static GateWs gate_ws(void* ws, int n, int K, int N) {
  const long n32 = (n + 31) / 32 * 32;
  GateWs w;
  w.wq = reinterpret_cast<unsigned char*>(ws);
  w.eq = w.wq + align256(4L * N * K);
  w.zq = w.eq + align256(4L * n32 * K);
  w.wqT = w.zq + align256(4L * n32 * N);
  w.eqT = w.wqT + align256(4L * N * K);
  w.zqT = w.eqT + align256(4L * n32 * K);
  return w;
}
static bool dual_add(SplitDual& q, const float* src, unsigned char* dst, unsigned char* dstT, int rows, int cols) {
  if (q.nseg >= 4 || (rows & 31) || (cols & 31) || ((reinterpret_cast<uintptr_t>(src) | reinterpret_cast<uintptr_t>(dst) | reinterpret_cast<uintptr_t>(dstT)) & 15))
    return false;
  q.src[q.nseg] = src; q.dst[q.nseg] = dst; q.dstT[q.nseg] = dstT; q.rows[q.nseg] = rows; q.cols[q.nseg] = cols;
  q.first[q.nseg + 1] = q.first[q.nseg] + (long)(rows >> 5) * (cols >> 5);
  ++q.nseg;
  return true;
}
static int launch_gate_stage(SplitDual& q, hipStream_t s) {
  long blocks = q.first[q.nseg];
  if (blocks == 0) return LIREC_OK;
  q.fmt16c = g_gemm_mode == 3 ? 1 : 0;
  double bytes = 0.0;
  for (int i = 0; i < q.nseg; ++i) bytes += 4.0 * q.rows[i] * (double)q.cols[i] * (q.fmt16c ? (q.dstT[i] ? 2.0 : 1.5) : (q.dstT[i] ? 3.0 : 2.0));
  if (blocks > 8192) blocks = 8192;
  const int pi = prof_start(PS_GATE_STAGE, s);
  lirec::launch(split_q32b_dual_kernel, dim3((unsigned)blocks), dim3(256), 0, s, q);
  prof_stop(pi, s, 0.0, bytes);
  LIREC_CHECK_LAUNCH();
  return LIREC_OK;
}
static bool gate_p3_ok(int n, int K, int N, int split) {
  if (g_gemm_mode == 3 && ((n | K | N) & 63)) return false;
  return (n & 127) == 0 && (N & 127) == 0 && N % 96 == 0 && K % 96 == 0 && split % 96 == 0 && (K - split) % 96 == 0 && K / 96 >= 8 &&
         !(g_ablate & 16);
}
static int p3_pick_ni(int M, int N, bool n128_ok) {
  const long cus = p2_grid(), tm = M / 128;
  const long r3 = (tm * (N / 96) + cus - 1) / cus, r4 = (tm * (N / 128) + cus - 1) / cus;
  return (n128_ok && r4 * 4 < r3 * 3) ? 4 : 3;
}
static unsigned p3_setup(GemmGroup& g, int BM, int BN, bool persistent = true) {
  int tn = 0;
  for (int i = 0; i < g.nprob; ++i) tn += g.p[i].N / BN;
  g.p3_tm = g.p[0].M / BM; g.p3_tn = tn; g.p3_xm = 0;
  double best = 0.0;
  for (int xm = 1; xm <= 8; xm *= 2) {
    const int xn = 8 / xm;
    if (g.p3_tm % xm || tn % xn) continue;
    const double cost = (double)(g.p3_tm / xm) * BM + (double)(tn / xn) * BN;
    if (g.p3_xm == 0 || cost < best) { best = cost; g.p3_xm = xm; }
  }
  const long tiles = (long)g.p3_tm * tn;
  const int cus = p2_grid();
  const long grid = (tiles < cus || !persistent) ? tiles : cus;
  if (grid & 7) g.p3_xm = 0;
  return (unsigned)grid;
}

int64_t lirec_gate_ws_bytes(int32_t n, int32_t K, int32_t N) {
  if (n < 0 || K < 0 || N < 0) return -1;
  const int64_t n32 = (n + 31) / 32 * 32;
  return 2 * (align256(4L * N * K) + align256(4L * n32 * K) + align256(4L * n32 * N));
}

int lirec_gate_stage_weights(const float* Wg, int32_t n, int32_t K, int32_t N, void* ws, int64_t ws_bytes, lirec_stream_t stream) {
  if (!Wg || n < 0 || K < 1 || N < 1) return LIREC_EINVAL;
  if (!gate_q32_ok(n, K, N, K, ws, ws_bytes) || (reinterpret_cast<uintptr_t>(Wg) & 15) != 0) return LIREC_EINVAL;
  const GateWs w = gate_ws(ws, n, K, N);
  SplitDual q;
  memset(&q, 0, sizeof(q));
  if (!dual_add(q, Wg, w.wq, w.wqT, N, K)) return LIREC_EINVAL;
  return launch_gate_stage(q, (hipStream_t)stream);
}

int lirec_gate_fwd_ws(const float* EE, int64_t ldee, const float* Wg, const float* bg, int32_t n, int32_t K,
                      int32_t N, float* G, int64_t ldg, const lirec_dropout* drop, void* ws, int64_t ws_bytes,
                      int32_t weights_staged, lirec_stream_t stream) {
  if (!EE || !Wg || !G || n < 0 || K < 1 || N < 1) return LIREC_EINVAL;
  if (!gate_q32_ok(n, K, N, ldee, ws, ws_bytes) || ((reinterpret_cast<uintptr_t>(EE) | reinterpret_cast<uintptr_t>(Wg)) & 15) != 0)
    return weights_staged ? LIREC_EINVAL : lirec_gate_fwd(EE, ldee, Wg, bg, n, K, N, G, ldg, drop, stream);
  hipStream_t s = (hipStream_t)stream;
  const GateWs w = gate_ws(ws, n, K, N);
  SplitDual q;
  memset(&q, 0, sizeof(q));
  if ((!weights_staged && !dual_add(q, Wg, w.wq, w.wqT, N, K)) || !dual_add(q, EE, w.eq, w.eqT, n, K)) return LIREC_EINVAL;
  int rc = launch_gate_stage(q, s);
  if (rc) return rc;
  GemmGroup g;
  memset(&g, 0, sizeof(g));
  g.nprob = 1;
  GemmProblem p = make_problem();
  p.A = reinterpret_cast<const float*>(w.eq); p.lda = K;
  p.B = reinterpret_cast<const float*>(w.wq); p.ldb = K;
  p.bias = bg; p.C = G; p.ldc = ldg;
  p.M = n; p.N = N; p.K = K; p.epi = EPI_DROP_RELU;
  set_dropout(p, drop, drop ? drop->site : LIREC_SITE_GATE, 0);
  g.p[0] = p;
  if (gate_p3_ok(n, K, N, K / 2)) {
    const int ni = p3_pick_ni(n, N, (N & 127) == 0);
    const unsigned grid = p3_setup(g, 128, 32 * ni);
    const int pi = prof_start(PS_GATE_FWD, s);
    g.onepass = g_gemm_mode == 3;
    launch_p3_fwd(ni, dim3(grid), s, g);
    prof_stop(pi, s, 2.0 * n * (double)N * K, 0.0);
    LIREC_CHECK_LAUNCH();
    return LIREC_OK;
  }
  return launch_p2<L_NT>(g, s, PS_GATE_FWD, nullptr, 1);
}

int lirec_gate_bwd_ws(const float* dZg, int64_t lddzg, const float* EE, int64_t ldee, const float* Wg,
                      int32_t n, int32_t K, int32_t N, int32_t split,
                      const float* Tn, int64_t ldtn, float* dWg, float* dbg, float* dEE, int64_t lddee,
                      int32_t acc_first, const lirec_dropout* drop, int32_t site_ctx, int32_t site_ints,
                      int32_t parts, void* ws, int64_t ws_bytes, int32_t rows_staged, lirec_stream_t stream) {
  if (!dZg || !EE || !Wg || !Tn || !dWg || !dbg || !dEE || n < 0 || K < 1 || N < 1 || split < 0 || split > K || parts < 0 ||
      (parts > 2 && parts != 4))
    return LIREC_EINVAL;
  const bool q32 = gate_q32_ok(n, K, N, ldee, ws, ws_bytes) && lddzg == N && 2 * split == K &&
                   (gate_p3_ok(n, K, N, split) || (split & 255) == 0) && (reinterpret_cast<uintptr_t>(dZg) & 15) == 0;
  if (!q32) {
    if (parts == 4) return LIREC_OK;
    return lirec_gate_bwd_parts(dZg, lddzg, EE, ldee, Wg, n, K, N, split, Tn, ldtn, dWg, dbg, dEE, lddee, acc_first, drop, site_ctx,
                                site_ints, parts, stream);
  }
  hipStream_t s = (hipStream_t)stream;
  int rc = LIREC_OK;
  const GateWs w = gate_ws(ws, n, K, N);
  if (!rows_staged) {
    SplitDual q;
    memset(&q, 0, sizeof(q));
    if (!dual_add(q, dZg, w.zq, w.zqT, n, N)) return LIREC_EINVAL;
    rc = launch_gate_stage(q, s);
    if (rc || parts == 4) return rc;
  } else if (parts == 4) {
    return LIREC_OK;
  }
  const bool p3 = gate_p3_ok(n, K, N, split);
  if (parts != 2) {
    if (p3 && ldee == K) {
      GemmGroup gw;
      memset(&gw, 0, sizeof(gw));
      gw.nprob = 1;
      GemmProblem p = make_problem();
      p.A = reinterpret_cast<const float*>(w.zqT); p.lda = n;
      p.B = reinterpret_cast<const float*>(w.eqT); p.ldb = n;
      p.C = dWg; p.ldc = K;
      p.M = N; p.N = K; p.K = n;
      p.beta = grad_beta(); p.dbias_set = g_grad_overwrite; p.dbias = dbg;
      gw.p[0] = p;
      ow_note_group(gw);
      const unsigned grid = p3_setup(gw, 128, 96, !(g_ablate & 32768));
      const int pi = prof_start(PS_GATE_DW, s);
      gw.onepass = g_gemm_mode == 3;
      launch_p3_wgrad(dim3(grid), s, gw);
      prof_stop(pi, s, 2.0 * n * (double)N * K, 0.0);
      LIREC_CHECK_LAUNCH();
    } else {
      rc = lirec_gate_bwd_parts(dZg, lddzg, EE, ldee, Wg, n, K, N, split, Tn, ldtn, dWg, dbg, dEE, lddee, acc_first, drop, site_ctx,
                                site_ints, 1, stream);
    }
  }
  if (rc || parts == 1) return rc;
  GemmGroup gd;
  memset(&gd, 0, sizeof(gd));
  gd.nprob = 2;
  for (int h = 0; h < 2; ++h) {
    const int c0 = h == 0 ? 0 : split, nc = h == 0 ? split : K - split;
    GemmProblem p = make_problem();
    p.A = reinterpret_cast<const float*>(w.zq); p.lda = N;
    if (p3) { p.B = reinterpret_cast<const float*>(w.wqT + 4096L * (c0 / 32) * (g_gemm_mode == 3 ? N / 64 : N / 32)); p.ldb = N; }
    else { p.B = reinterpret_cast<const float*>(w.wq + 4096L * (c0 / 32)); p.ldb = K; }
    p.C = dEE + c0; p.ldc = lddee;
    p.M = n; p.N = nc; p.K = N;
    p.epi = EPI_TANH_BWD; p.aux = Tn + c0; p.ldaux = ldtn;
    p.beta = (h == 0 && acc_first) ? 1.f : 0.f;
    set_dropout(p, drop, h == 0 ? site_ctx : site_ints, 0);
    gd.p[h] = p;
  }
  if (p3) {
    const int ni = p3_pick_ni(n, K, (split & 127) == 0 && ((K - split) & 127) == 0);
    const unsigned grid = p3_setup(gd, 128, 32 * ni);
    const int pi = prof_start(PS_GATE_DEE, s);
    gd.onepass = g_gemm_mode == 3;
    launch_p3_dgrad(ni, dim3(grid), s, gd);
    prof_stop(pi, s, 2.0 * n * (double)N * K, 0.0);
    LIREC_CHECK_LAUNCH();
    return LIREC_OK;
  }
  return launch_p2<L_NN>(gd, s, PS_GATE_DEE, nullptr, 1);
}

static int linear_fwd_problem(const lirec_linear_fwd_args& v, GemmProblem& p) {
  if (!v.A || !v.W || !v.Y || v.n < 0 || v.K < 1 || v.N < 1) return LIREC_EINVAL;
  p = make_problem();
  p.A = v.A; p.lda = v.lda; p.B = v.W; p.ldb = v.K; p.bias = v.b; p.C = v.Y; p.ldc = v.ldy;
  p.M = v.n; p.N = v.N; p.K = v.K; p.epi = EPI_STORE;
  return LIREC_OK;
}

int lirec_linear_fwd_group(const lirec_linear_fwd_args* v, int32_t count, lirec_stream_t stream) {
  if (!v || count < 1 || count > LIREC_MAX_PROB) return LIREC_EINVAL;
  GemmGroup g; g.nprob = count;
  for (int i = 0; i < count; ++i) {
    const int rc = linear_fwd_problem(v[i], g.p[i]);
    if (rc) return rc;
  }
  return launch_gemm(L_NT, g, (hipStream_t)stream, PS_LINEAR_FWD);
}

int lirec_linear_fwd(const float* A, int64_t lda, const float* W, const float* b, int32_t n, int32_t K,
                     int32_t N, float* Y, int64_t ldy, lirec_stream_t stream) {
  const lirec_linear_fwd_args v = {A, lda, W, b, Y, ldy, n, K, N, 0};
  return lirec_linear_fwd_group(&v, 1, stream);
}

int lirec_linear_bwd_group(const lirec_linear_bwd_args* v, int32_t count, lirec_stream_t stream) {
  if (!v || count < 1 || count > LIREC_MAX_PROB) return LIREC_EINVAL;
  hipStream_t s = (hipStream_t)stream;
  if ((g_ablate & 131072) && v[0].parts != 2) lirec::launch(spin_kernel, dim3(1), dim3(64), 0, s, 200000LL);
  GemmGroup gw, gd;
  gw.nprob = 0; gd.nprob = 0;
  for (int i = 0; i < count; ++i) {
    const lirec_linear_bwd_args& a = v[i];
    if (!a.dY || !a.A || !a.W || !a.dW || !a.db || a.n < 0 || a.K < 1 || a.N < 1 || a.parts < 0 || a.parts > 2) return LIREC_EINVAL;
    if (a.dA && a.mode != 0 && !a.act) return LIREC_EINVAL;
    if (a.parts != 2) {
      GemmProblem w = make_problem();
      w.A = a.dY; w.lda = a.lddy; w.B = a.A; w.ldb = a.lda; w.C = a.dW; w.ldc = a.K;
      w.M = a.N; w.N = a.K; w.K = a.n; w.beta = grad_beta(); w.dbias_set = g_grad_overwrite; w.dbias = a.db;
      gw.p[gw.nprob++] = w;
    }
    if (!a.dA || a.parts == 1) continue;
    GemmProblem p = make_problem();
    p.A = a.dY; p.lda = a.lddy; p.B = a.W; p.ldb = a.K; p.C = a.dA; p.ldc = a.ldda;
    p.M = a.n; p.N = a.K; p.K = a.N;
    p.beta = a.accumulate ? 1.f : 0.f;
    const float pd = a.drop.p;
    if (a.mode == 1) {
      p.epi = EPI_RELU_BWD; p.aux = a.act; p.ldaux = a.ldact;
      p.drop_scale = (pd > 0.f) ? (float)(1.0 / (1.0 - (double)pd)) : 1.f;
    } else if (a.mode == 2) {
      p.epi = EPI_TANH_BWD; p.aux = a.act; p.ldaux = a.ldact;
      set_dropout(p, &a.drop, a.drop.site2, 0);
    } else {
      p.epi = EPI_STORE;
    }
    gd.p[gd.nprob++] = p;
  }
  int rc = launch_gemm(L_TN, gw, s, PS_LINEAR_DW);
  if (rc || gd.nprob == 0) return rc;
  return launch_gemm(L_NN, gd, s, PS_LINEAR_DA);
}

int lirec_linear_bwd(const float* dY, int64_t lddy, const float* A, int64_t lda, const float* W,
                     int32_t n, int32_t K, int32_t N, float* dW, float* db,
                     float* dA, int64_t ldda, int32_t mode, const float* act, int64_t ldact,
                     int32_t accumulate, const lirec_dropout* drop, lirec_stream_t stream) {
  lirec_linear_bwd_args v;
  memset(&v, 0, sizeof(v));
  v.dY = dY; v.lddy = lddy; v.A = A; v.lda = lda; v.W = W; v.n = n; v.K = K; v.N = N; v.dW = dW; v.db = db;
  v.dA = dA; v.ldda = ldda; v.mode = mode; v.act = act; v.ldact = ldact; v.accumulate = accumulate; v.parts = 0;
  if (drop) v.drop = *drop;
  return lirec_linear_bwd_group(&v, 1, stream);
}

int lirec_margin_loss(const lirec_margin_loss_args* a, lirec_stream_t stream) {
  if (!a || !a->ints || !a->y || a->B < 1 || a->T < 1 || a->C < 1 || a->sample < 0 || a->sample > 2) return LIREC_EINVAL;
  const bool probs_only = a->sample == 2;
  if (probs_only ? !(a->probs_out || a->sel_out) : (!a->d_ints || !a->loss || !a->partial)) return LIREC_EINVAL;
  if (a->rels && (!a->r || (!probs_only && !a->d_rels) || a->NR < 1)) return LIREC_EINVAL;
  if (a->rels && a->rels_mean_valid && a->T != 1) return LIREC_EINVAL;
  if (a->sample && a->tr_correct) return LIREC_EINVAL;
  if (a->batch_divisor < 0.f || a->rels_divisor < 0.f) return LIREC_EINVAL;
  hipStream_t s = (hipStream_t)stream;
  const int NR1 = a->rels ? a->NR + 1 : 0;
  const size_t shm = ((size_t)a->T * a->C + (size_t)a->T * NR1 + 16 + 4 + 2 * (size_t)a->T + a->C) * sizeof(float);
  if (shm > 160 * 1024) return LIREC_EINVAL;
  const int pi = prof_start(PS_LOSS, s);
  lirec::launch(margin_loss_kernel, dim3(a->B), dim3(256), shm, s, *a);
  if (!probs_only && !a->arrive) {
    LIREC_CHECK_LAUNCH();
    lirec::launch(loss_finalize_kernel, dim3(1), dim3(256), 0, s, (const float*)a->partial, 2 * a->B, a->loss);
  }
  prof_stop(pi, s, 0.0, 8.0 * a->B * a->T * ((double)a->C + (a->rels ? a->NR : 0)));
  LIREC_CHECK_LAUNCH();
  return LIREC_OK;
}

int lirec_heads_loss_fwd_bwd(const lirec_linear_fwd_args* heads, const lirec_linear_bwd_args* back, int32_t n_heads,
                             const lirec_margin_loss_args* loss, lirec_stream_t stream) {
  if (!heads || n_heads < 1 || n_heads > LIREC_MAX_PROB || (loss && !back)) return LIREC_EINVAL;
  int rc = lirec_linear_fwd_group(heads, n_heads, stream);
  if (rc || !loss) return rc;
  bool ints_ok = false;
  for (int h = 0; h < n_heads; ++h) ints_ok = ints_ok || heads[h].Y == loss->ints;
  if (!ints_ok) return LIREC_EINVAL;
  rc = lirec_margin_loss(loss, stream);
  if (rc) return rc;
  lirec_linear_bwd_args b[LIREC_MAX_PROB];
  for (int h = 0; h < n_heads; ++h) { b[h] = back[h]; b[h].parts = 2; }
  return lirec_linear_bwd_group(b, n_heads, stream);
}

int lirec_ce_loss(const float* ints, int64_t ld_ints, const float* rels, int64_t ld_rels,
                  const int32_t* y, const int32_t* r, const float* class_w,
                  int32_t B, int32_t C, int32_t NR, float* d_ints, int64_t ld_dints,
                  float* d_rels, int64_t ld_drels, float* loss, float* partial,
                  float den_ints, float den_rels, const float* dens_dev, lirec_stream_t stream) {
  if (!ints || !y || !d_ints || !loss || !partial || B < 1 || C < 1 || den_ints < 0.f || den_rels < 0.f) return LIREC_EINVAL;
  if (rels && (!r || !d_rels || NR < 1)) return LIREC_EINVAL;
  hipStream_t s = (hipStream_t)stream;
  const int nblk = rels ? 2 * B : B;
  lirec::launch(ce_loss_kernel, dim3(nblk), dim3(256), 0, s, ints, (long)ld_ints, rels, (long)ld_rels, y, r,
                     class_w, B, C, NR, d_ints, (long)ld_dints, d_rels, (long)ld_drels, partial, den_ints, den_rels, dens_dev);
  LIREC_CHECK_LAUNCH();
  lirec::launch(loss_finalize_kernel, dim3(1), dim3(256), 0, s, (const float*)partial, nblk, loss);
  LIREC_CHECK_LAUNCH();
  return LIREC_OK;
}

static bool adam_aligned(const float* p, const float* g, const float* m, const float* v) {
  return ((reinterpret_cast<uintptr_t>(p) | reinterpret_cast<uintptr_t>(g) | reinterpret_cast<uintptr_t>(m) |
           reinterpret_cast<uintptr_t>(v)) & 15) == 0;
}

int lirec_adam_step(float* p, const float* g, float* m, float* v, int64_t n, int32_t step,
                    float lr, float beta1, float beta2, float eps, float weight_decay,
                    float grad_scale, const int64_t* step_dev, lirec_stream_t stream) {
  if (!p || !g || !m || !v || n < 0 || (step < 1 && !step_dev)) return LIREC_EINVAL;
  if (!adam_aligned(p, g, m, v)) return LIREC_EINVAL;
  if (step < 1) step = 1;
  if (n == 0) return LIREC_OK;
  const double bc1 = 1.0 - pow((double)beta1, (double)step);
  const double bc2 = 1.0 - pow((double)beta2, (double)step);
// ... 162 lines not shown
```

lirec_amd/model.py:

```python
from __future__ import annotations

import ctypes as C

import torch
import torch.nn as nn

from . import ops
from ._lib import SITE_E_CTX, SITE_E_INTS, SITE_GATE, SITE_H1_CTX, SITE_H1_INTS, LirecError
from .config import opt

__all__ = ['Modalities', 'MidFusionMultiClip', 'MidFusionMultiClipMaxTracks', 'GatingUnit',
           'MultiTaskCrossEntropyLoss', 'MultiTaskMaxMargin', 'MaxMarginCrossEntropyLoss',
           'MarginLoss', 'MarginTrackRelsLoss', 'create_model']


_SIDE_LANES = {}


def _ptr(t: torch.Tensor, col: int = 0) -> int:
    return t.data_ptr() + 4 * col


def _dev_tensor(t, device, dtype):
    if not torch.is_tensor(t):
# ... 300 lines not shown
    def _run_forward(self, X, mask, n, R, clamp):
        dev, J = X.device, opt.joint_dim
        Rp1 = X.shape[1]
        D = X.shape[2]
        st = {'X': X, 'mask': mask, 'n': n, 'R': R, 'clamp': clamp, 'seed': self._cur_seed, 'seed_dev': self._seed_dev,
              'train': self.training, 'inters': None, 'rels': None}
        has_i, has_c, has_g = self._has_ints, self._has_ctx, self._has_gate
        self.last_layer1_planes = False
        if not self.training or not getattr(self, '_defer_side_join', False):
            self.join_side_streams()
        Wi = self._segs_i.width if has_i else 0
        Wc = self._segs_c.width if has_c else 0
        pieces = getattr(self, '_pieces_cur', None)
        pc = ops.make_pieces(pieces['clip'], pieces['track'], pieces['index'], opt.text_dim, opt.visual_dim,
                             pieces.get('clip_rows'), pieces.get('track_rows')) if pieces is not None else None
        pq = pc if (pc is not None and has_i and has_c and getattr(opt, 'pieces_q32b', False) and getattr(opt, 'layer1_planes', False)
                    and self.training and not pieces.get('requires_grad')) else None
        pre = self._take_prestaged(X, mask, n, R) if (has_i and has_c and pieces is None) else None
        st['prestaged'] = pre is not None
        EE = ops.new((n, Wc + Wi), dtype=torch.float32, device=dev)
        Tn = ops.new_like(EE)
        ldee = Wc + Wi
        if has_i:
            mods, segs = self._mods_i, self._segs_i
            H1 = ops.new((n, segs.n * J), dtype=torch.float32, device=dev)
            W1, b1 = zip(*[self._W(a) for a, _ in mods])
            W2, b2 = zip(*[self._W(b) for _, b in mods])
            pl = pre['planes_i'] if pre is not None else self._planes_buffer(X, n, segs, J)
            args_i = ops.embed_fwd_args(X, D, (1, Rp1, 0), n, J, segs, W1, b1, W2, b2, H1, _ptr(EE, Wc), ldee,
                                        _ptr(Tn, Wc), ldee, 1, self._dropout(SITE_H1_INTS, SITE_E_INTS), planes=pl, pieces=pq,
                                        rows_staged=pre is not None, W1q=self._w1q_of(mods, pl))
            st['H1_i'], st['planes_i'] = H1, pl
        if has_c:
            mods, segs = self._mods_c, self._segs_c
            H1 = ops.new((n * R, segs.n * J), dtype=torch.float32, device=dev)
            Hbar = ops.new((n, segs.n * J), dtype=torch.float32, device=dev)
            fsc = ops.new((n,), dtype=torch.float32, device=dev)
            W1, b1 = zip(*[self._W(a) for a, _ in mods])
            W2, b2 = zip(*[self._W(b) for _, b in mods])
            cmp = pre['cmp'] if pre is not None else (ops.compact_rows(mask, n, R) if opt.compact_ctx_rows else None)
            if cmp is None and mask.dtype != torch.float32:
                mask = mask.to(torch.float32)
            if cmp is not None:
                mask = None
            st['mask'] = mask
            pl = pre['planes_c'] if pre is not None else self._planes_buffer(X, n * R, segs, J)
            if pre is not None:
                self.last_layer1_planes = True
            W_c = segs.n * J
            hb = None
            if self.training and getattr(opt, 'h1_sign_bits', True) and R <= 64 and W_c % 4 == 0:
                hb = ops.new(max(ops.hbits_bytes(n * R, W_c), 16), dtype=torch.uint8, device=dev)
            args_c = ops.embed_fwd_args(X, D, (R, Rp1, 1), n * R, J, segs, W1, b1, W2, b2, H1, _ptr(EE), ldee, _ptr(Tn), ldee,
                                        1, self._dropout(SITE_H1_CTX, SITE_E_CTX), pool=(mask, R, clamp, Hbar, fsc, cmp),
                                        planes=pl, pieces=pq, hbits=hb, rows_staged=pre is not None, W1q=self._w1q_of(mods, pl))
            st['Hbar'], st['fsc'], st['cmp'], st['planes_c'], st['hbits_c'] = Hbar, fsc, cmp, pl, hb
            st['H1_c'] = H1 if (hb is None or self.debug_keep_state) else None
        st['EE'], st['Tn'] = EE, Tn
        G = None
        if has_g:
            Wg, bg = self._W_gate()
            N = Wg.shape[0]
            G = ops.new((n, N), dtype=torch.float32, device=dev)
            st['G'] = G
            gws, w_side = None, None
            if self.training and getattr(opt, 'gate_q32', True) and n % 32 == 0:
                gws = ops.new(ops.gate_ws_bytes(n, ldee, N), dtype=torch.uint8, device=dev)
                lane = self._wgrad_lane()
                if lane is not None and getattr(opt, 'gate_stage_on_side', True):
                    side_h, main = C.c_void_p(lane[0].cuda_stream), ops.current_stream_handle()
                    if not getattr(self, '_bucket0_on_side', False):
                        ops.stream_wait(side_h, main)
                    self._bucket0_on_side = False
                    with ops.on_stream(side_h):
                        if ops.gate_stage_weights(Wg, n, ldee, N, gws):
                            w_side = (main, side_h)
            st['gate_ws'] = gws
            st['w_side_staged'] = w_side is not None
        deferred_join = None
        if self.training and getattr(self, '_defer_side_join', False) and has_g and w_side is None:
            lane0 = self._wgrad_lane()
            if lane0 is not None:
                deferred_join = (ops.current_stream_handle(), C.c_void_p(lane0[0].cuda_stream))
        st['pieces'] = pieces if pq is None else None
        st['pieces_gather'] = pq if (pq is not None and isinstance(pieces['clip'], ops.Q32Block)) else None
        if pq is None and pieces is not None and isinstance(pieces['clip'], ops.Q32Block):
            raise LirecError('q32b piece tables serve training steps on the q32b layer-1 kernels only (opt.pieces_q32b, opt.layer1_planes)')
        if pieces is not None and pq is None:
            nc, nt = pieces['clip'].shape[0], pieces['track'].shape[0]
            zs = [ops.new((m, 2 * J), dtype=torch.float32, device=dev) for m in (nc, nt, nc, nt)]
            ops.embed_l1_indexed([args_i, args_c], pc, [zs[0], zs[2]], [zs[1], zs[3]])
            if has_g and w_side is not None:
                ops.stream_wait(*w_side)
            elif deferred_join is not None:
                ops.stream_wait(*deferred_join)
            ops.embed_fwd2(ops.with_parts(args_i, 3), ops.with_parts(args_c, 3))
            if has_g:
                ops.gate_fwd(EE, ldee, Wg, bg, n, ldee, N, G, N, self._dropout(SITE_GATE), ws=st['gate_ws'],
                             weights_staged=w_side is not None)
        else:
            def layers(parts):
                if has_i and has_c:
                    ops.embed_fwd2(ops.with_parts(args_i, parts), ops.with_parts(args_c, parts)) if parts else ops.embed_fwd2(args_i, args_c)
                elif has_i:
                    ops.embed_fwd(args=ops.with_parts(args_i, parts) if parts else args_i)
                elif has_c:
                    ops.embed_fwd(args=ops.with_parts(args_c, parts) if parts else args_c)
            if has_g and w_side is not None:
                layers(1)
                ops.stream_wait(*w_side)
                layers(2)
            elif deferred_join is not None:
                layers(1)
                ops.stream_wait(*deferred_join)
                layers(2)
            else:
                layers(0)
            if has_g:
                ops.gate_fwd(EE, ldee, Wg, bg, n, ldee, N, G, N, self._dropout(SITE_GATE), ws=st['gate_ws'],
                             weights_staged=w_side is not None)
        heads = []
        if has_i:
            Wo, bo = self._W('out_ints')
            inters = ops.new((n, Wo.shape[0]), dtype=torch.float32, device=dev)
            if has_g:
                heads.append((_ptr(st['G']), st['G'].shape[1], Wo, bo, n, st['G'].shape[1], Wo.shape[0], inters, Wo.shape[0]))
            else:
                heads.append((_ptr(EE, Wc), ldee, Wo, bo, n, Wi, Wo.shape[0], inters, Wo.shape[0]))
            st['inters'] = inters
        if has_c:
            Wo, bo = self._W('out_ctx')
            rels = ops.new((n, Wo.shape[0]), dtype=torch.float32, device=dev)
            heads.append((_ptr(EE), ldee, Wo, bo, n, Wc, Wo.shape[0], rels, Wo.shape[0]))
            st['rels'] = rels
        if heads:
            ops.linear_fwd_group(heads)
        return st

    def _W_gate(self):
        return self.gates_ints.fc_out.weight, self.gates_ints.fc_out.bias

    def _wgrad_lane(self, which: int = 0):
        if not getattr(opt, 'wgrad_side_stream', True):
            return None
        if getattr(self, '_sides', None) is None:
            self._sides = {}
        if which not in self._sides:
            prio = 0
            key = (str(self._flat.device), prio, which)
            if key not in _SIDE_LANES:
                lane = (torch.cuda.Stream(device=self._flat.device, priority=prio), ops.Context())
                with lane[1]:
                    ops.ensure_scratch(self._flat.device, (128 if which == 0 else 64) << 20)
                _SIDE_LANES[key] = lane
            self._sides[which] = _SIDE_LANES[key]
        return self._sides[which]

    def _run_backward(self, st, d_inters, d_rels, want_dx=False, want_dp=(False, False)):
        if want_dx and (not torch.is_tensor(st['X']) or st.get('pieces') is not None or st.get('pieces_gather') is not None
                        or st.get('prestaged')):
            raise LirecError('the features\' gradient is formed for a feature block (a tensor) only -- not for q32b storage, '
                             'piece tables or prestaged rows')
        want_dp = any(want_dp)
        if want_dp and st.get('pieces') is None:
            raise LirecError('the piece tables\' gradient is formed on the once-per-piece path only (lirec_embed_l1_indexed)')
        self.flat_grads(attach=True)
        pieces = st.get('pieces')
        lane = self._wgrad_lane()
        main = ops.current_stream_handle() if lane is not None else None
        side_h = C.c_void_p(lane[0].cuda_stream) if lane is not None else None
        lane2 = self._wgrad_lane(1) if lane is not None else None
        side2_h = C.c_void_p(lane2[0].cuda_stream) if lane2 is not None else None

        core = ops.get_gemm_mode()

        def on_side2(fn):
            ops.stream_wait_many([side2_h, side_h], main)
            with ops.on_stream(side2_h), lane2[1]:
                ops.set_gemm_mode(core)
                fn()

        def on_side(fn):
            ops.stream_wait(side_h, main)
            with ops.on_stream(side_h), lane[1]:
                ops.set_gemm_mode(core)
                fn()

        defer = bool(getattr(self, '_defer_side_join', False)) and lane is not None and self._has_gate and self._has_ints \
            and self.grad_sync is None and st.get('train', False) and bool(getattr(opt, 'adam_on_side_stream', True)) \
            and bool(getattr(opt, 'wgrad_side_stream', True))

        def join_side():
            if lane is not None and not defer:
                ops.stream_wait(main, side_h)
            if lane2 is not None:
                ops.stream_wait(main, side2_h)
        X, n, R, J = st['X'], st['n'], st['R'], opt.joint_dim
        dev = X.device
        Rp1, D = X.shape[1], X.shape[2]
        has_i, has_c, has_g = self._has_ints, self._has_ctx, self._has_gate
        Wi = self._segs_i.width if has_i else 0
        Wc = self._segs_c.width if has_c else 0
        ldee = Wc + Wi
        EE, Tn = st['EE'], st['Tn']
        p = float(opt.dropout) if st['train'] else 0.0
        seed = st['seed']
        drop = lambda s1, s2=0: ops.make_dropout(seed, p, s1, s2, st.get('seed_dev'))
        dEE = ops.new((n, ldee), dtype=torch.float32, device=dev)
        if d_inters is not None:
            d_inters = d_inters.reshape(n, -1).contiguous().float()
        if d_rels is not None:
            d_rels = d_rels.reshape(n, -1).contiguous().float()

        heads = []
        if has_c:
            Wo, _ = self._W('out_ctx')
            if d_rels is None:
                d_rels = ops.zero_(ops.new((n, Wo.shape[0]), dtype=torch.float32, device=dev))
            heads.append((d_rels, d_rels.shape[1], _ptr(EE), ldee, Wo, n, Wc, Wo.shape[0],
                          self._g('out_ctx.weight'), self._g('out_ctx.bias'), _ptr(dEE), ldee,
                          0 if has_g else 2, None if has_g else _ptr(Tn), ldee, 0, drop(0, SITE_E_CTX)))
        dZg = None
        if has_i:
            Wo, _ = self._W('out_ints')
            if d_inters is None:
                d_inters = ops.zero_(ops.new((n, Wo.shape[0]), dtype=torch.float32, device=dev))
            if has_g:
                G = st['G']
                N = G.shape[1]
                dZg = ops.new_like(G)
                heads.append((d_inters, d_inters.shape[1], _ptr(G), N, Wo, n, N, Wo.shape[0],
                              self._g('out_ints.weight'), self._g('out_ints.bias'), _ptr(dZg), N,
                              1, _ptr(G), N, 0, drop(SITE_GATE)))
            else:
                heads.append((d_inters, d_inters.shape[1], _ptr(EE, Wc), ldee, Wo, n, Wi, Wo.shape[0],
                              self._g('out_ints.weight'), self._g('out_ints.bias'), _ptr(dEE, Wc), ldee,
                              2, _ptr(Tn, Wc), ldee, 0, drop(0, SITE_E_INTS)))
        one_fork = bool(heads) and lane is not None and has_i and has_g
        if heads and lane is not None:
            if not one_fork:
                on_side(lambda: ops.linear_bwd_group(heads, parts=1))
            ops.linear_bwd_group(heads, parts=2)
        elif heads:
            ops.linear_bwd_group(heads)
        if has_i and has_g:
            G = st['G']
            N = G.shape[1]
            Wg, _ = self._W_gate()
            gate = lambda parts: ops.gate_bwd(dZg, N, EE, ldee, Wg, n, ldee, N, Wc, Tn, ldee,
                                              self._g('gates_ints.fc_out.weight'), self._g('gates_ints.fc_out.bias'),
                                              dEE, ldee, has_c, drop(0), SITE_E_CTX, SITE_E_INTS, parts=parts,
                                              ws=st.get('gate_ws'), rows_staged=staged)
            staged = False
            if st.get('gate_ws') is not None and lane is not None:
                gate(4)
                staged = True
            if one_fork:
                on_side(lambda: (ops.linear_bwd_group(heads, parts=1), gate(1)))
                gate(2)
            else:
                gate(0)
        if self.grad_sync is not None:
            self.grad_sync.bucket_ready(0, also=side_h)
        args_i = args_c = None
        adam = self.__dict__.pop('_dw1_adam', None)
        if want_dx:
            adam = None
        if adam is not None and not (has_i and has_c and pieces is None and st.get('planes_i') is not None
                                     and st.get('planes_c') is not None and self.grad_sync is None):
            adam = None
        self._dw1_adam_applied = adam is not None
        if has_i:
            mods, segs = self._mods_i, self._segs_i
            ws_i = ops.new(ops.workspace_bytes(n, segs.n, J) // 4, dtype=torch.float32, device=dev)
            args_i = ops.embed_bwd_args(X, D, (1, Rp1, 0), n, J, segs, [self._W(b)[0] for _, b in mods], st['H1_i'],
                                        _ptr(dEE, Wc), ldee,
                                        [self._g(a + '.weight') for a, _ in mods], [self._g(a + '.bias') for a, _ in mods],
                                        [self._g(b + '.weight') for _, b in mods], [self._g(b + '.bias') for _, b in mods],
                                        ws_i, drop(SITE_H1_INTS), planes=st.get('planes_i'), pieces=st.get('pieces_gather'), adam=adam)
        if has_c:
            mods, segs = self._mods_c, self._segs_c
            ws_c = ops.new(ops.workspace_bytes(n * R + n, segs.n, J) // 4, dtype=torch.float32, device=dev)
            args_c = ops.embed_bwd_args(X, D, (R, Rp1, 1), n * R, J, segs, [self._W(b)[0] for _, b in mods], st['H1_c'],
                                        _ptr(dEE), ldee,
                                        [self._g(a + '.weight') for a, _ in mods], [self._g(a + '.bias') for a, _ in mods],
                                        [self._g(b + '.weight') for _, b in mods], [self._g(b + '.bias') for _, b in mods],
                                        ws_c, drop(SITE_H1_CTX),
                                        pool=(st['mask'], R, st['clamp'], st['Hbar'], st['fsc'], st['cmp']),
                                        planes=st.get('planes_c'), hbits=st.get('hbits_c'), pieces=st.get('pieces_gather'), adam=adam)

        def run(parts, which=None):
            if which is None and args_i is not None and args_c is not None:
                ops.embed_bwd2(ops.with_parts(args_i, parts), ops.with_parts(args_c, parts))
            else:
                for a in ((args_i, args_c) if which is None else (which,)):
                    if a is not None:
                        ops.embed_bwd(args=ops.with_parts(a, parts))
        if lane2 is not None:
            on_side2(lambda: run(1))
        elif lane is not None:
            on_side(lambda: run(1))
        else:
            run(1)
        if self.grad_sync is not None:
            self.grad_sync.bucket_ready(1, also=side2_h if lane2 is not None else side_h)
        dClip = dTrack = None
        if pieces is not None:
            run(3)
            ops.embed_bwd(args=ops.with_parts(args_c, 5))
            pc = ops.make_pieces(pieces['clip'], pieces['track'], pieces['index'], opt.text_dim, opt.visual_dim)
            nc1, nt1 = pieces['clip'].shape[0], pieces['track'].shape[0]
            ldp = (nc1 + 2 * nt1 + 3) // 4 * 4
            Ps = [ops.new((n * ldp,), dtype=torch.float32, device=dev), ops.new((n * R * ldp,), dtype=torch.float32, device=dev)]
            Ss = [ops.new(((nc1 + nt1) * 2 * J,), dtype=torch.float32, device=dev) for _ in range(2)]
            ops.embed_dw1_indexed([args_i, args_c], pc, Ps, Ss)
            if want_dp:
                dClip = ops.new(pieces['clip'].shape, dtype=torch.float32, device=dev)
                dTrack = ops.new(pieces['track'].shape, dtype=torch.float32, device=dev)
                W1 = [[self._W(m1)[0] for m1, _ in mods] for mods in (self._mods_i, self._mods_c)]
                ops.embed_dx_indexed([args_i, args_c], Ss, W1, pc, dClip, dTrack)
        else:
            run(2)
        dX = None
        if want_dx:
            dX = ops.new(X.shape, dtype=X.dtype, device=dev)
            hs = [(a, mods) for a, mods in ((args_i, getattr(self, '_mods_i', None)), (args_c, getattr(self, '_mods_c', None)))
                  if a is not None]
            ops.embed_dx([a for a, _ in hs], [[self._W(m1)[0] for m1, _ in mods] for _, mods in hs], dX)
        join_side()
        if self.grad_sync is not None:
            self.grad_sync.bucket_ready(2)
        self._side_after_backward = (side_h, main) if (lane is not None and has_g and has_i) else None
        self._side_unjoined = defer
        return dX, dClip, dTrack

    def first_layer_range(self):
        from .parallel import stage_of
# ... 555 lines not shown
```

lirec_amd/ops.py:

```python
from __future__ import annotations

import ctypes as C
import threading

import torch

from . import _lib
from ._lib import (Dropout, FusedAdamArgs, EmbedBwdArgs, EmbedDxArgs, EmbedDxIndexedArgs, EmbedFwdArgs, EvalArgs, LinearBwdArgs,
                   LinearFwdArgs, MarginLossArgs, Pieces, RowSel, check, lib)


class _ThreadCell(threading.local):
    value = None

    def __getitem__(self, i):
        return self.value

    def __setitem__(self, i, v):
        self.value = v


_stream_override = _ThreadCell()


# ... 178 lines not shown
    return Q32Block(out, t.shape)


def to_q16b(t, out=None, k64=False):
    if t.dtype == torch.bfloat16:
        t = t.float()
    assert t.is_cuda and t.dtype == torch.float32 and t.is_contiguous()
    D = t.shape[-1]
    rows = t.numel() // D
    need = max(int(lib().lirec_q16b_bytes(rows, D)), 256)
    if out is None:
        out = torch.empty(need, dtype=torch.uint8, device=t.device)
    assert out.dtype == torch.uint8 and out.is_cuda and out.numel() >= need and out.data_ptr() % 256 == 0
    if k64:
        check(lib().lirec_to_q16c(_p(t), D, rows, D, _p(out), _stream()), 'lirec_to_q16c')
    else:
        check(lib().lirec_to_q16b(_p(t), D, rows, D, _p(out), _stream()), 'lirec_to_q16b')
    return Q32Block(out, t.shape, planes=1, k64=k64)


def to_q16c(t, out=None):
    return to_q16b(t, out=out, k64=True)


def to_q16(t, out=None):
    return to_q16b(t, out=out, k64=get_gemm_mode() == 3)


def make_dropout(seed: int, p: float, site: int = 0, site2: int = 0, seed_dev=None) -> Dropout:
    return Dropout(int(seed) & 0xFFFFFFFFFFFFFFFF, float(p), int(site), int(site2),
                   None if seed_dev is None else seed_dev.data_ptr())


class Segments:

    def __init__(self, in_off, in_dim, out_dim):
        self.in_off, self.in_dim, self.out_dim = list(in_off), list(in_dim), list(out_dim)
        self.n = len(self.in_off)
        assert 1 <= self.n <= _lib.MAX_SEG

    @property
    def width(self):
        return sum(self.out_dim)


def _fill(arr, vals):
    for i, v in enumerate(vals):
        arr[i] = v


def embed_fwd_args(X, ldx, sel, rows, J, segs: Segments, W1, b1, W2, b2, H1, Z2, ldz2, Tn, ldtn, epilogue, drop,
                   pool=None, planes=None, pieces=None, hbits=None, rows_staged=False, W1q=None):
    a = EmbedFwdArgs()
    a.rows_staged = int(bool(rows_staged))
    if W1q is not None:
        _fill(a.W1q, [int(w) for w in W1q])
    if hbits is not None:
        a.hbits = _p(hbits)
    if pieces is not None:
        a.pieces = C.cast(C.pointer(pieces), C.c_void_p)
        a._pieces_ref = pieces
    if planes is not None:
        a.planes, a.planes_bytes = _p(planes), planes.numel() * planes.element_size()
    if pool is not None:
        mask, R, clamp, Hbar, fscale = pool[:5]
        a.mask, a.R, a.clamp_zero, a.Hbar, a.fscale = _p(mask), R, int(clamp), _p(Hbar), _p(fscale)
        if len(pool) > 5 and pool[5] is not None:
            a.rowmap, a.cstart, a.count = (_p(t) for t in pool[5][:3])
            a.wts = _p(pool[5][3]) if len(pool[5]) > 3 else None
    a.X, a.ldx = _p(X), ldx
    a.x_bf16 = int(X.dtype == torch.bfloat16)
    a.x_q32 = X.x_q32 if isinstance(X, Q32Block) else 0
    _fill(a.W1, [_p(w) for w in W1]); _fill(a.b1, [_p(w) for w in b1])
    _fill(a.W2, [_p(w) for w in W2]); _fill(a.b2, [_p(w) for w in b2])
    a.H1, a.Z2, a.ldz2 = _p(H1), Z2, ldz2
    a.Tn, a.ldtn = Tn, ldtn
    _fill(a.in_off, segs.in_off); _fill(a.in_dim, segs.in_dim); _fill(a.out_dim, segs.out_dim)
    a.rows, a.nseg, a.J, a.epilogue = rows, segs.n, J, epilogue
    a.sel = RowSel(*sel)
    a.drop = drop
    return a


def embed_fwd(*args, **kw):
    a = kw['args'] if 'args' in kw else embed_fwd_args(*args, **kw)
    check(lib().lirec_embed_fwd(C.byref(a), _stream()), 'lirec_embed_fwd')


def embed_fwd2(a, b):
    check(lib().lirec_embed_fwd2(C.byref(a), C.byref(b), _stream()), 'lirec_embed_fwd2')


def embed_bwd_args(X, ldx, sel, rows, J, segs: Segments, W2, H1, dZ2, lddz2, dW1, db1, dW2, db2, workspace, drop,
                   pool=None, planes=None, parts=0, hbits=None, pieces=None, adam=None):
    a = EmbedBwdArgs()
    a.parts = int(parts)
    if adam is not None:
        a.adam = C.cast(C.pointer(adam), C.c_void_p)
        a._adam_ref = adam
    if pieces is not None:
        a.pieces = C.cast(C.pointer(pieces), C.c_void_p)
        a._pieces_ref = pieces
    if hbits is not None:
        a.hbits = _p(hbits)
    if planes is not None:
        a.planes, a.planes_bytes = _p(planes), planes.numel() * planes.element_size()
    if pool is not None:
        mask, R, clamp, Hbar, fscale = pool[:5]
        a.mask, a.R, a.clamp_zero, a.Hbar, a.fscale = _p(mask), R, int(clamp), _p(Hbar), _p(fscale)
        if len(pool) > 5 and pool[5] is not None:
            a.rowmap, a.cstart, a.count = (_p(t) for t in pool[5][:3])
            a.wts = _p(pool[5][3]) if len(pool[5]) > 3 else None
    a.X, a.ldx = _p(X), ldx
    a.x_bf16 = int(X.dtype == torch.bfloat16)
    a.x_q32 = X.x_q32 if isinstance(X, Q32Block) else 0
    _fill(a.W2, [_p(w) for w in W2])
    a.H1, a.dZ2, a.lddz2 = (_p(H1) if H1 is not None else None), dZ2, lddz2
    _fill(a.dW1, [_p(w) for w in dW1]); _fill(a.db1, [_p(w) for w in db1])
    _fill(a.dW2, [_p(w) for w in dW2]); _fill(a.db2, [_p(w) for w in db2])
    a.workspace, a.workspace_bytes = _p(workspace), workspace.numel() * workspace.element_size()
    _fill(a.in_off, segs.in_off); _fill(a.in_dim, segs.in_dim); _fill(a.out_dim, segs.out_dim)
    a.rows, a.nseg, a.J = rows, segs.n, J
    a.sel = RowSel(*sel)
    a.drop = drop
    a._refs = (X, H1, workspace, planes, pool, hbits)
    return a


def make_pieces(clip, track, index, text_dim, visual_dim, clip_rows=None, track_rows=None):
    assert index.is_cuda and index.dtype == torch.int32 and index.is_contiguous()
    if isinstance(clip, Q32Block):
        assert isinstance(track, Q32Block) and clip.shape[1] == text_dim + visual_dim
        pc = Pieces(None, clip.shape[1], clip.shape[0] - 1, None, track.shape[1], track.shape[0] - 1, _p(index),
                    text_dim, visual_dim, track.shape[1])
        pc.clip_q, pc.track_q = _p(clip), _p(track)
        if clip_rows is not None:
            assert clip_rows.dtype == torch.int32 and track_rows.dtype == torch.int32 and clip_rows.is_cuda and track_rows.is_cuda
            pc.clip_rows, pc.track_rows = _p(clip_rows), _p(track_rows)
        pc._refs = (clip, track, index, clip_rows, track_rows)
        return pc
    assert clip.is_cuda and clip.dtype == torch.float32 and track.dtype == torch.float32
    assert clip.is_contiguous() and track.is_contiguous() and clip.shape[1] == text_dim + visual_dim
    return Pieces(_p(clip), clip.shape[1], clip.shape[0] - 1, _p(track), track.shape[1], track.shape[0] - 1, _p(index),
                  text_dim, visual_dim, track.shape[1])


def embed_l1_indexed(heads, pieces, zclips, ztrks):
    n = len(heads)
    hp = (C.POINTER(EmbedFwdArgs) * n)(*[C.pointer(h) for h in heads])
    zc = (C.c_void_p * n)(*[_p(z) for z in zclips])
    zt = (C.c_void_p * n)(*[_p(z) for z in ztrks])
    check(lib().lirec_embed_l1_indexed(hp, n, C.byref(pieces), zc, zt, _stream()), 'lirec_embed_l1_indexed')


def embed_dw1_indexed(heads, pieces, Ps, Ss):
    n = len(heads)
    hp = (C.POINTER(EmbedBwdArgs) * n)(*[C.pointer(h) for h in heads])
    pp = (C.c_void_p * n)(*[_p(z) for z in Ps])
    sp = (C.c_void_p * n)(*[_p(z) for z in Ss])
    check(lib().lirec_embed_dw1_indexed(hp, n, C.byref(pieces), pp, sp, _stream()), 'lirec_embed_dw1_indexed')


def fused_adam_args(p, g, m, v, n_params, step, lr, beta1, beta2, eps, weight_decay, grad_scale=1.0, step_dev=None, wq=None, wq_first=0):
    for t in (p, g, m, v):
        assert t.is_cuda and t.dtype == torch.float32 and t.is_contiguous() and t.numel() == p.numel()
    a = FusedAdamArgs(_p(p), _p(g), _p(m), _p(v), _p(wq) if wq is not None else None, int(wq_first), p.numel(), int(n_params),
                int(step), float(lr), float(beta1), float(beta2), float(eps), float(weight_decay), float(grad_scale),
                None if step_dev is None else step_dev.data_ptr())
    a._refs = (p, g, m, v, wq, step_dev)
    return a


def with_parts(a, parts):
# ... 14 lines not shown
    check(lib().lirec_embed_bwd2(C.byref(a), C.byref(b), _stream()), 'lirec_embed_bwd2')


def embed_dx(heads, W1, dX):
    assert dX.is_cuda and dX.is_contiguous() and dX.dim() == 3 and dX.dtype in (torch.float32, torch.bfloat16)
    a = EmbedDxArgs()
    a.nh = len(heads)
    for h, (b, ws) in enumerate(zip(heads, W1)):
        a.heads[h] = C.pointer(b)
        _fill(a.W1[h], [_p(w) for w in ws])
    a.out_bf16 = int(dX.dtype == torch.bfloat16)
    a.dX, a.ldx = _p(dX), dX.shape[2]
    a.n, a.rp1, a.D = dX.shape[0], dX.shape[1], dX.shape[2]
    check(lib().lirec_embed_dx(C.byref(a), _stream()), 'lirec_embed_dx')


def embed_dx_indexed(heads, S, W1, pieces, dClip, dTrack):
    for t in (dClip, dTrack):
        assert t.is_cuda and t.is_contiguous() and t.dim() == 2 and t.dtype == torch.float32
    a = EmbedDxIndexedArgs()
    a.nh = len(heads)
    for h, (b, s, ws) in enumerate(zip(heads, S, W1)):
        a.heads[h] = C.pointer(b)
        a.S[h] = _p(s)
        _fill(a.W1[h], [_p(w) for w in ws])
    a.pieces = C.pointer(pieces)
    a.dClip, a.ld_clip = _p(dClip), dClip.shape[1]
    a.dTrack, a.ld_track = _p(dTrack), dTrack.shape[1]
    check(lib().lirec_embed_dx_indexed(C.byref(a), _stream()), 'lirec_embed_dx_indexed')


_MASK_DTYPES = {torch.float32: 0, torch.int64: 1, torch.float64: 2}


def compact_rows(mask, n, R, out=None):
    dev = mask.device
    assert mask.is_contiguous() and mask.numel() == n * R and mask.dtype in _MASK_DTYPES, (mask.dtype, mask.shape)
    if out is not None:
        rowmap, cstart, count, wts = out
        assert rowmap.numel() == n * R and cstart.numel() == n + 1
    else:
        rowmap = new(n * R, dtype=torch.int32, device=dev)
        cstart = new(2 * n + 1, dtype=torch.int32, device=dev)[:n + 1]
        count = new(1, dtype=torch.int32, device=dev)
        wts = new(n * R, dtype=torch.float32, device=dev)
    check(lib().lirec_compact_rows2(_p(mask), _MASK_DTYPES[mask.dtype], n, R, _p(rowmap), _p(cstart), _p(count), _p(wts),
                                    _stream()), 'lirec_compact_rows2')
    return rowmap, cstart, count, wts


def workspace_bytes(rows, nseg, J):
    return int(lib().lirec_workspace_bytes(rows, nseg, J))


def hbits_bytes(rows, W):
    return int(lib().lirec_hbits_bytes(int(rows), int(W)))


def planes_bytes(rows, dsum, J, gathered=False, bf16=False):
    return int(lib().lirec_planes_bytes(rows, dsum, J, 1 if bf16 else (2 if gathered else 0)))


def pool_fwd(Z2, ldz, mask, n, R, W, clamp, Tn, ldtn, E, lde, drop):
    check(lib().lirec_pool_fwd(_p(Z2), ldz, _p(mask), n, R, W, int(clamp), Tn, ldtn, E, lde, C.byref(drop), _stream()),
          'lirec_pool_fwd')


def pool_bwd(dP, lddp, mask, n, R, W, clamp, dZ2, lddz):
    check(lib().lirec_pool_bwd(dP, lddp, _p(mask), n, R, W, int(clamp), _p(dZ2), lddz, _stream()), 'lirec_pool_bwd')


def gate_ws_bytes(n, K, N):
    return int(lib().lirec_gate_ws_bytes(int(n), int(K), int(N)))


def gate_stage_weights(Wg, n, K, N, ws) -> bool:
    rc = lib().lirec_gate_stage_weights(_p(Wg), n, K, N, _p(ws), ws.numel() * ws.element_size(), _stream())
    if rc == _lib.LIREC_EINVAL:
        return False
    check(rc, 'lirec_gate_stage_weights')
    return True


def gate_fwd(EE, ldee, Wg, bg, n, K, N, G, ldg, drop, ws=None, weights_staged=False):
    if ws is not None:
        check(lib().lirec_gate_fwd_ws(_p(EE), ldee, _p(Wg), _p(bg), n, K, N, _p(G), ldg, C.byref(drop), _p(ws),
                                      ws.numel() * ws.element_size(), int(weights_staged), _stream()), 'lirec_gate_fwd_ws')
        return
    check(lib().lirec_gate_fwd(_p(EE), ldee, _p(Wg), _p(bg), n, K, N, _p(G), ldg, C.byref(drop), _stream()),
          'lirec_gate_fwd')


def gate_bwd(dZg, lddzg, EE, ldee, Wg, n, K, N, split, Tn, ldtn, dWg, dbg, dEE, lddee, acc_first, drop,
             site_ctx, site_ints, parts=0, ws=None, rows_staged=False):
    if ws is not None:
        check(lib().lirec_gate_bwd_ws(_p(dZg), lddzg, _p(EE), ldee, _p(Wg), n, K, N, split, _p(Tn), ldtn, _p(dWg), _p(dbg),
                                      _p(dEE), lddee, int(acc_first), C.byref(drop), site_ctx, site_ints, int(parts), _p(ws),
                                      ws.numel() * ws.element_size(), int(rows_staged), _stream()), 'lirec_gate_bwd_ws')
        return
    check(lib().lirec_gate_bwd_parts(_p(dZg), lddzg, _p(EE), ldee, _p(Wg), n, K, N, split, _p(Tn), ldtn, _p(dWg), _p(dbg),
                                     _p(dEE), lddee, int(acc_first), C.byref(drop), site_ctx, site_ints, int(parts), _stream()),
          'lirec_gate_bwd_parts')


def linear_fwd(A, lda, W, b, n, K, N, Y, ldy):
    check(lib().lirec_linear_fwd(A, lda, _p(W), _p(b), n, K, N, _p(Y), ldy, _stream()), 'lirec_linear_fwd')


def linear_fwd_group(items):
    arr = (LinearFwdArgs * len(items))()
    for v, (A, lda, W, b, n, K, N, Y, ldy) in zip(arr, items):
        v.A, v.lda, v.W, v.b, v.Y, v.ldy, v.n, v.K, v.N = A, lda, _p(W), _p(b), _p(Y), ldy, n, K, N
    check(lib().lirec_linear_fwd_group(arr, len(items), _stream()), 'lirec_linear_fwd_group')


def linear_bwd_group(items, parts=0):
    arr = (LinearBwdArgs * len(items))()
    for v, (dY, lddy, A, lda, W, n, K, N, dW, db, dA, ldda, mode, act, ldact, accumulate, drop) in zip(arr, items):
        v.dY, v.lddy, v.A, v.lda, v.W = _p(dY), lddy, A, lda, _p(W)
        v.dW, v.db, v.dA, v.ldda, v.act, v.ldact = _p(dW), _p(db), dA, ldda, act, ldact
        v.n, v.K, v.N, v.mode, v.accumulate, v.parts = n, K, N, mode, int(accumulate), int(parts)
        v.drop = drop
    check(lib().lirec_linear_bwd_group(arr, len(items), _stream()), 'lirec_linear_bwd_group')


def linear_bwd(dY, lddy, A, lda, W, n, K, N, dW, db, dA, ldda, mode, act, ldact, accumulate, drop):
    check(lib().lirec_linear_bwd(_p(dY), lddy, A, lda, _p(W), n, K, N, _p(dW), _p(db), dA, ldda, mode, act, ldact,
                                 int(accumulate), C.byref(drop), _stream()), 'lirec_linear_bwd')


_ARRIVE = {}


def _arrive_counter(dev):
    key = (dev.type, dev.index, current_stream_handle().value)
    if key not in _ARRIVE:
        _ARRIVE[key] = torch.zeros(1, dtype=torch.int32, device=dev)
    return _ARRIVE[key]


def margin_loss(ints, rels, mem, w, y, r, g, sel, B, T, Cc, NR, margin, lymbda, max_neg, tr_correct,
                mask_inplace, rels_mean_valid, loader_types=False, sample=0, sample_seed=0, sample_seed_dev=None,
                want_probs=False, heads=None, back=None, divisors=None, y_stride=1):
    dev = ints.device
    probs_only = sample == 2
    d_ints = None if probs_only else new((B * T, Cc), dtype=torch.float32, device=dev)
    d_rels = new((B * T, NR), dtype=torch.float32, device=dev) if (rels is not None and not probs_only) else None
    loss = None if probs_only else new(1, dtype=torch.float32, device=dev)
    partial = None if probs_only else new(2 * B + 2, dtype=torch.float32, device=dev)
    sel_out = new(B, dtype=torch.int32, device=dev)
    probs = new((B, T), dtype=torch.float32, device=dev) if (want_probs or probs_only) else None
    a = MarginLossArgs()
    a.ints, a.ld_ints = _p(ints), ints.stride(0)
    a.rels, a.ld_rels = _p(rels), (rels.stride(0) if rels is not None else 0)
    a.mem, a.w, a.y, a.r, a.g, a.sel = _p(mem), _p(w), _p(y), _p(r), _p(g), _p(sel)
    a.d_ints, a.ld_dints = _p(d_ints), Cc
    a.d_rels, a.ld_drels = _p(d_rels), NR
    a.loss, a.partial, a.sel_out = _p(loss), _p(partial), _p(sel_out)
    a.B, a.T, a.C, a.NR = B, T, Cc, NR
    a.margin, a.lymbda = margin, lymbda
    a.max_neg, a.tr_correct, a.mask_inplace, a.rels_mean_valid = int(max_neg), int(tr_correct), int(mask_inplace), int(rels_mean_valid)
    a.loader_types = int(bool(loader_types))
    a.sample, a.sample_seed = int(sample), int(sample_seed) & 0xFFFFFFFFFFFFFFFF
    a.sample_seed_dev = _p(sample_seed_dev)
    a.probs_out = _p(probs)
    a.arrive = None if probs_only else _p(_arrive_counter(dev))
    _set_divisors(a, divisors, dev)
    a.y_stride = int(y_stride)
    if loader_types:
        assert all(t is None or t.dtype == torch.float64 for t in (mem, w)) and \
            all(t is None or t.dtype == torch.int64 for t in (y, r, g))
    else:
        assert all(t is None or t.dtype == torch.float32 for t in (mem, w)) and \
            all(t is None or t.dtype == torch.int32 for t in (y, r, g))
    if heads is None:
        check(lib().lirec_margin_loss(C.byref(a), _stream()), 'lirec_margin_loss')
        return loss, d_ints, d_rels, sel_out, probs
    assert back is not None and len(back) == len(heads) and not probs_only
    fwd = (LinearFwdArgs * len(heads))()
    for v, (A, lda, W, b, n, K, N, Y, ldy) in zip(fwd, heads):
        v.A, v.lda, v.W, v.b, v.Y, v.ldy, v.n, v.K, v.N = A, lda, _p(W), _p(b), _p(Y), ldy, n, K, N
    bwd = (LinearBwdArgs * len(back))()
    for v, (dY, lddy, A, lda, W, n, K, N, dW, db, dA, ldda, mode, act, ldact, accumulate, drop) in zip(bwd, back):
        dYt = {'ints': d_ints, 'rels': d_rels}[dY]
        v.dY, v.lddy, v.A, v.lda, v.W = _p(dYt), lddy, A, lda, _p(W)
        v.dW, v.db, v.dA, v.ldda, v.act, v.ldact = _p(dW), _p(db), dA, ldda, act, ldact
        v.n, v.K, v.N, v.mode, v.accumulate, v.parts = n, K, N, mode, int(accumulate), 2
        v.drop = drop
    check(lib().lirec_heads_loss_fwd_bwd(fwd, bwd, len(heads), C.byref(a), _stream()), 'lirec_heads_loss_fwd_bwd')
    return loss, d_ints, d_rels, sel_out, probs


def _set_divisors(a, divisors, dev):
    a.batch_divisor = a.rels_divisor = 0.0
    a.divisors_dev = None
    if divisors is None:
        return
    if torch.is_tensor(divisors):
        assert divisors.device == dev and divisors.dtype == torch.float32 and divisors.numel() >= 2 and divisors.is_contiguous()
        a.divisors_dev = _p(divisors)
    else:
        a.batch_divisor, a.rels_divisor = float(divisors[0]), float(divisors[1])


def ce_loss(ints, rels, y, r, class_w, B, Cc, NR, divisors=None):
    dev = ints.device
# ... 173 lines not shown
```

Before: 78860.

## Fuse gate-input bf16x3 staging into producer GEMM epilogues via LDS sink

The embed layer-2 forward GEMM (tanh+dropout epilogue) and the linear head backward GEMM (relu-bwd epilogue) now also write their output tiles as split bf16 hi/lo planes, both row-major and transposed, into the gate workspace. They do this through a per-wave LDS tile that reuses the k-loop stage buffers. The gate forward and backward can then skip their separate row-staging passes, saving a read and re-quantisation of EE and dZg. In exchange the epilogue does extra LDS traffic and global stores, sink-attached problems are excluded from K-splitting, and new ABI entry points are added.

```diff
diff --git a/include/lirec_hip.h b/include/lirec_hip.h
--- a/include/lirec_hip.h
+++ b/include/lirec_hip.h
@@ -172,6 +172,14 @@
                       int32_t acc_first, const lirec_dropout* drop, int32_t site_ctx, int32_t site_ints,
                       int32_t parts, void* ws, int64_t ws_bytes, int32_t rows_staged, lirec_stream_t stream);
 
+int lirec_embed_fwd_ws(const lirec_embed_fwd_args* a, void* ws, int64_t ws_bytes, int32_t gate_n, int32_t gate_K, int32_t gate_N,
+                       int32_t* staged, lirec_stream_t stream);
+int lirec_embed_fwd2_ws(const lirec_embed_fwd_args* a, const lirec_embed_fwd_args* b, void* ws, int64_t ws_bytes, int32_t gate_n,
+                        int32_t gate_K, int32_t gate_N, int32_t* staged, lirec_stream_t stream);
+int lirec_gate_fwd_ws2(const float* EE, int64_t ldee, const float* Wg, const float* bg, int32_t n, int32_t K,
+                       int32_t N, float* G, int64_t ldg, const lirec_dropout* drop, void* ws, int64_t ws_bytes,
+                       int32_t weights_staged, int32_t rows_staged, lirec_stream_t stream);
+
 int lirec_linear_fwd(const float* A, int64_t lda, const float* W, const float* b, int32_t n, int32_t K,
                      int32_t N, float* Y, int64_t ldy, lirec_stream_t stream);
 int lirec_linear_bwd(const float* dY, int64_t lddy, const float* A, int64_t lda, const float* W,
@@ -192,6 +200,8 @@
   lirec_dropout drop;
 } lirec_linear_bwd_args;
 int lirec_linear_bwd_group(const lirec_linear_bwd_args* v, int32_t count, lirec_stream_t stream);
+int lirec_linear_bwd_group_ws(const lirec_linear_bwd_args* v, int32_t count, int32_t stage_head, void* ws, int64_t ws_bytes,
+                              int32_t gate_n, int32_t gate_K, int32_t gate_N, int32_t* staged, lirec_stream_t stream);
 
 typedef struct {
   float* ints; int64_t ld_ints;
diff --git a/lirec_amd/_lib.py b/lirec_amd/_lib.py
--- a/lirec_amd/_lib.py
+++ b/lirec_amd/_lib.py
@@ -151,6 +151,10 @@
     'lirec_embed_bwd2': (_i32, [C.POINTER(EmbedBwdArgs), C.POINTER(EmbedBwdArgs), _vp]),
     'lirec_embed_dx': (_i32, [C.POINTER(EmbedDxArgs), _vp]),
     'lirec_embed_dx_indexed': (_i32, [C.POINTER(EmbedDxIndexedArgs), _vp]),
+    'lirec_embed_fwd_ws': (_i32, [C.POINTER(EmbedFwdArgs), _vp, _i64, _i32, _i32, _i32, C.POINTER(_i32), _vp]),
+    'lirec_embed_fwd2_ws': (_i32, [C.POINTER(EmbedFwdArgs), C.POINTER(EmbedFwdArgs), _vp, _i64, _i32, _i32, _i32, C.POINTER(_i32), _vp]),
+    'lirec_gate_fwd_ws2': (_i32, [_vp, _i64, _vp, _vp, _i32, _i32, _i32, _vp, _i64, C.POINTER(Dropout), _vp, _i64, _i32, _i32, _vp]),
+    'lirec_linear_bwd_group_ws': (_i32, [C.POINTER(LinearBwdArgs), _i32, _i32, _vp, _i64, _i32, _i32, _i32, C.POINTER(_i32), _vp]),
     'lirec_linear_fwd_group': (_i32, [C.POINTER(LinearFwdArgs), _i32, _vp]),
     'lirec_linear_bwd_group': (_i32, [C.POINTER(LinearBwdArgs), _i32, _vp]),
     'lirec_compact_rows': (_i32, [_vp, _i32, _i32, _vp, _vp, _vp, _vp]),
diff --git a/lirec_amd/csrc/gemm.hpp b/lirec_amd/csrc/gemm.hpp
--- a/lirec_amd/csrc/gemm.hpp
+++ b/lirec_amd/csrc/gemm.hpp
@@ -33,6 +33,7 @@
   const int* srow;
   const void* A_lo; const void* B_lo;
   unsigned char* xq_out; long ld_xq;
+  unsigned char* sq; unsigned char* sqT; int s_rbn, s_cbn, s_cb0;
 };
 
 struct AdamFuse {
@@ -87,6 +88,7 @@
   float slab_cost, reduce_cost;
   GemmProblem p[LIREC_MAX_PROB];
 };
+static_assert(sizeof(GemmGroup) <= 4096, "GemmGroup travels as a kernel argument: 4 KiB at most");
 struct GemmMeta { int site; int tag; };
 
 inline bool gemm_problem_is_vec(int layout, const GemmProblem& p) {
@@ -328,9 +330,24 @@
   return c;
 }
 
-template <int WM, int WN, int EPI>
+typedef float f32x2 __attribute__((ext_vector_type(2)));
+typedef __bf16 bf16x2 __attribute__((ext_vector_type(2)));
+__device__ __forceinline__ void split4(const f32x4 v, uint2& hi, uint2& lo) {
+  const f32x2 v01 = {v[0], v[1]}, v23 = {v[2], v[3]};
+  const bf16x2 h01 = __builtin_convertvector(v01, bf16x2), h23 = __builtin_convertvector(v23, bf16x2);
+  const unsigned w01 = __builtin_bit_cast(unsigned, h01), w23 = __builtin_bit_cast(unsigned, h23);
+  const f32x2 f01 = {__builtin_bit_cast(float, w01 << 16), __builtin_bit_cast(float, w01 & 0xffff0000u)};
+  const f32x2 f23 = {__builtin_bit_cast(float, w23 << 16), __builtin_bit_cast(float, w23 & 0xffff0000u)};
+  const f32x2 r01 = v01 - f01, r23 = v23 - f23;
+  const bf16x2 l01 = __builtin_convertvector(r01, bf16x2), l23 = __builtin_convertvector(r23, bf16x2);
+  hi = make_uint2(w01, w23);
+  lo = make_uint2(__builtin_bit_cast(unsigned, l01), __builtin_bit_cast(unsigned, l23));
+}
+
+template <int WM, int WN, int EPI, bool SINK = false>
 __device__ __forceinline__ void gemm_epilogue_kind(const GemmProblem& p, const f32x16 (&acc)[WM][WN], int m0, int n0,
-                                                   int wm0, int wn0, int lane, int M, bool have_rid = false, int rid_lane = 0) {
+                                                   int wm0, int wn0, int lane, int M, bool have_rid = false, int rid_lane = 0,
+                                                   float* lds = nullptr) {
   constexpr bool USES_RND = (EPI == EPI_DROP_RELU || EPI == EPI_TANH_DROP || EPI == EPI_TANH_BWD);
   constexpr bool USES_AUX = (EPI == EPI_RELU_BWD || EPI == EPI_TANH_BWD);
   const int l31 = lane & 31, lh = lane >> 5;
@@ -353,6 +370,7 @@
     for (int j = 0; j < WN; ++j) {
       const int col = n0 + wn0 + 32 * j + l31;
       const bool colok = col < N;
+      const bool sink_blk = SINK && (n0 + wn0 + 32 * j) < N && (m0 + wm0 + 32 * i) < M;
       float axp[PRE_AUX ? 16 : 1];
       if constexpr (PRE_AUX) {
 #pragma unroll
@@ -423,8 +441,36 @@
             v *= keep ? f * p.drop_scale : 0.f;
           }
           if (ok[jj]) *cptr[jj] = v;
+          if constexpr (SINK) { if (sink_blk) lds[(8 * q + 4 * lh + jj) * 33 + l31] = v; }
         }
         __asm__ volatile("" ::: "memory");
+      }
+      if constexpr (SINK) {
+        if (sink_blk) {
+          __builtin_amdgcn_fence(__ATOMIC_RELEASE, "wavefront");
+          __builtin_amdgcn_wave_barrier();
+          __builtin_amdgcn_fence(__ATOMIC_ACQUIRE, "wavefront");
+          const long rb = (m0 + wm0 + 32 * i) >> 5, cb = p.s_cb0 + ((n0 + wn0 + 32 * j) >> 5);
+          const int r8 = lane >> 3, c4 = lane & 7;
+          unsigned char* d = p.sq + ((rb * p.s_cbn + cb) * 32 + r8) * 128 + c4 * 8;
+          unsigned char* dt = p.sqT + ((cb * p.s_rbn + rb) * 32 + r8) * 128 + c4 * 8;
+#pragma unroll
+          for (int ps = 0; ps < 4; ++ps) {
+            const float* row = lds + (8 * ps + r8) * 33 + 4 * c4;
+            const float* colp = lds + (4 * c4) * 33 + 8 * ps + r8;
+            const f32x4 t = {row[0], row[1], row[2], row[3]};
+            const f32x4 w = {colp[0], colp[33], colp[66], colp[99]};
+            uint2 h, l;
+            split4(t, h, l);
+            *reinterpret_cast<uint2*>(d + 1024 * ps) = h;
+            *reinterpret_cast<uint2*>(d + 1024 * ps + 64) = l;
+            split4(w, h, l);
+            *reinterpret_cast<uint2*>(dt + 1024 * ps) = h;
+            *reinterpret_cast<uint2*>(dt + 1024 * ps + 64) = l;
+          }
+          __builtin_amdgcn_fence(__ATOMIC_RELEASE, "wavefront");
+          __builtin_amdgcn_wave_barrier();
+        }
       }
     }
   }
@@ -437,7 +483,8 @@
 
 template <int WM, int WN, int LAYOUT>
 __device__ __forceinline__ void gemm_epilogue(const GemmProblem& p, const f32x16 (&acc)[WM][WN], int m0, int n0,
-                                              int wm0, int wn0, int lane, int split, int M_eff, bool have_rid = false, int rid_lane = 0) {
+                                              int wm0, int wn0, int lane, int split, int M_eff, bool have_rid = false, int rid_lane = 0,
+                                              float* sink_lds = nullptr) {
   const int l31 = lane & 31, lh = lane >> 5;
   const int M = M_eff, N = p.N;
   if (p.ksplit > 1) {
@@ -457,10 +504,16 @@
   }
   if constexpr (LAYOUT == L_NT) {
     if (p.epi == EPI_DROP_RELU) gemm_epilogue_kind<WM, WN, EPI_DROP_RELU>(p, acc, m0, n0, wm0, wn0, lane, M, have_rid, rid_lane);
-    else if (p.epi == EPI_TANH_DROP) gemm_epilogue_kind<WM, WN, EPI_TANH_DROP>(p, acc, m0, n0, wm0, wn0, lane, M);
+    else if (p.epi == EPI_TANH_DROP) {
+      if (p.sq != nullptr && sink_lds != nullptr) gemm_epilogue_kind<WM, WN, EPI_TANH_DROP, true>(p, acc, m0, n0, wm0, wn0, lane, M, false, 0, sink_lds);
+      else gemm_epilogue_kind<WM, WN, EPI_TANH_DROP>(p, acc, m0, n0, wm0, wn0, lane, M);
+    }
     else gemm_epilogue_kind<WM, WN, EPI_STORE>(p, acc, m0, n0, wm0, wn0, lane, M);
   } else if constexpr (LAYOUT == L_NN) {
-    if (p.epi == EPI_RELU_BWD) gemm_epilogue_kind<WM, WN, EPI_RELU_BWD>(p, acc, m0, n0, wm0, wn0, lane, M);
+    if (p.epi == EPI_RELU_BWD) {
+      if (p.sq != nullptr && sink_lds != nullptr) gemm_epilogue_kind<WM, WN, EPI_RELU_BWD, true>(p, acc, m0, n0, wm0, wn0, lane, M, false, 0, sink_lds);
+      else gemm_epilogue_kind<WM, WN, EPI_RELU_BWD>(p, acc, m0, n0, wm0, wn0, lane, M);
+    }
     else if (p.epi == EPI_TANH_BWD) gemm_epilogue_kind<WM, WN, EPI_TANH_BWD>(p, acc, m0, n0, wm0, wn0, lane, M);
     else gemm_epilogue_kind<WM, WN, EPI_STORE>(p, acc, m0, n0, wm0, wn0, lane, M);
   } else {
diff --git a/lirec_amd/csrc/gemm_bf16x3.hpp b/lirec_amd/csrc/gemm_bf16x3.hpp
--- a/lirec_amd/csrc/gemm_bf16x3.hpp
+++ b/lirec_amd/csrc/gemm_bf16x3.hpp
@@ -9,19 +9,6 @@
 typedef short s16x4 __attribute__((ext_vector_type(4)));
 typedef short s16x8 __attribute__((ext_vector_type(8)));
 
-typedef float f32x2 __attribute__((ext_vector_type(2)));
-typedef __bf16 bf16x2 __attribute__((ext_vector_type(2)));
-__device__ __forceinline__ void split4(const f32x4 v, uint2& hi, uint2& lo) {
-  const f32x2 v01 = {v[0], v[1]}, v23 = {v[2], v[3]};
-  const bf16x2 h01 = __builtin_convertvector(v01, bf16x2), h23 = __builtin_convertvector(v23, bf16x2);
-  const unsigned w01 = __builtin_bit_cast(unsigned, h01), w23 = __builtin_bit_cast(unsigned, h23);
-  const f32x2 f01 = {__builtin_bit_cast(float, w01 << 16), __builtin_bit_cast(float, w01 & 0xffff0000u)};
-  const f32x2 f23 = {__builtin_bit_cast(float, w23 << 16), __builtin_bit_cast(float, w23 & 0xffff0000u)};
-  const f32x2 r01 = v01 - f01, r23 = v23 - f23;
-  const bf16x2 l01 = __builtin_convertvector(r01, bf16x2), l23 = __builtin_convertvector(r23, bf16x2);
-  hi = make_uint2(w01, w23);
-  lo = make_uint2(__builtin_bit_cast(unsigned, l01), __builtin_bit_cast(unsigned, l23));
-}
 
 __device__ __forceinline__ uint2 hi4(const f32x4 v) {
   const f32x2 v01 = {v[0], v[1]}, v23 = {v[2], v[3]};
@@ -361,7 +348,8 @@
   else if (interior) mainloop(std::false_type{}, std::false_type{});
   else mainloop(std::true_type{}, std::false_type{});
 
-  gemm_epilogue<WM, WN, LAYOUT>(p, acc, m0, n0, wm0, wn0, lane, tc.split, M);
+  static_assert((NTHR / 64) * 32 * 33 * 4 <= 2 * BUF, "the waves' sink tiles must fit the k-loop's stages");
+  gemm_epilogue<WM, WN, LAYOUT>(p, acc, m0, n0, wm0, wn0, lane, tc.split, M, false, 0, reinterpret_cast<float*>(smem) + wave * (32 * 33));
 
   if constexpr (LAYOUT == L_TN) {
     if (do_dbias) {
diff --git a/lirec_amd/csrc/lirec_hip.hip b/lirec_amd/csrc/lirec_hip.hip
--- a/lirec_amd/csrc/lirec_hip.hip
+++ b/lirec_amd/csrc/lirec_hip.hip
@@ -274,7 +274,7 @@
     t128 += (long)((p.M + 127) / 128) * ((p.N + 127) / 128);
     t64 += (long)((p.M + 63) / 64) * ((p.N + 63) / 64);
     mn_total += (long)p.M * p.N + (p.dbias ? p.M : 0);
-    splittable = splittable && p.K >= 512 && (p.epi == EPI_STORE || (p.rowmap == nullptr && p.dyn == nullptr && p.K >= 2048 &&
+    splittable = splittable && p.sq == nullptr && p.K >= 512 && (p.epi == EPI_STORE || (p.rowmap == nullptr && p.dyn == nullptr && p.K >= 2048 &&
                                                                      (g_ablate & 128)));
     any_epi = any_epi || p.epi != EPI_STORE;
     wide = wide && p.M >= 96 && p.N >= 96;
@@ -1167,7 +1167,45 @@
   return rc;
 }
 
-int lirec_embed_fwd(const lirec_embed_fwd_args* a, lirec_stream_t stream) {
+struct GateSink { void* ws; int64_t ws_bytes; int n, K, N; };
+static bool gate_q32_ok(int n, int K, int N, int64_t ldee, const void* ws, int64_t ws_bytes);
+struct GateWs { unsigned char* wq; unsigned char* eq; unsigned char* zq; unsigned char* wqT; unsigned char* eqT; unsigned char* zqT; };
+static GateWs gate_ws(void* ws, int n, int K, int N);
+static bool gate_sink_ok(const GateSink* k) {
+  return k && g_gemm_mode == 2 && !(g_ablate & 524288) && gate_q32_ok(k->n, k->K, k->N, k->K, k->ws, k->ws_bytes);
+}
+static bool attach_fwd_sink(GemmGroup* const* gs, int ng, const GateSink* k) {
+  if (!gate_sink_ok(k)) return false;
+  const float* base = nullptr;
+  for (int gi = 0; gi < ng; ++gi)
+    for (int i = 0; i < gs[gi]->nprob; ++i)
+      if (!base || gs[gi]->p[i].C < base) base = gs[gi]->p[i].C;
+  long c0[2 * LIREC_MAX_PROB], c1[2 * LIREC_MAX_PROB], sum = 0;
+  int np = 0;
+  for (int gi = 0; gi < ng; ++gi)
+    for (int i = 0; i < gs[gi]->nprob; ++i) {
+      const GemmProblem& p = gs[gi]->p[i];
+      const long off = p.C - base;
+      if (np >= 2 * LIREC_MAX_PROB || p.epi != EPI_TANH_DROP || p.M != k->n || p.ldc != k->K || p.rowmap || p.dyn || p.N < 32 || (p.N & 31) ||
+          (off & 31) || off + p.N > k->K)
+        return false;
+      for (int j = 0; j < np; ++j) if (off < c1[j] && c0[j] < off + p.N) return false;
+      c0[np] = off; c1[np] = off + p.N; ++np; sum += p.N;
+    }
+  if (sum != k->K) return false;
+  const GateWs w = gate_ws(k->ws, k->n, k->K, k->N);
+  for (int gi = 0; gi < ng; ++gi)
+    for (int i = 0; i < gs[gi]->nprob; ++i) {
+      GemmProblem& p = gs[gi]->p[i];
+      p.sq = w.eq; p.sqT = w.eqT; p.s_rbn = k->n >> 5; p.s_cbn = k->K >> 5; p.s_cb0 = (int)((p.C - base) >> 5);
+    }
+  return true;
+}
+static bool gate_sink_args_bad(const GateSink* k, const int32_t* staged) {
+  return !staged || k->ws_bytes < 0 || (!k->ws && k->ws_bytes != 0) || k->n < 0 || k->K < 1 || k->N < 1;
+}
+
+static int embed_fwd_impl(const lirec_embed_fwd_args* a, lirec_stream_t stream, const GateSink* sink, int32_t* staged) {
   GemmGroup g1, g2;
   int rc = embed_fwd_build(a, g1, g2);
   if (rc) return rc;
@@ -1178,10 +1216,25 @@
   if (a->parts == 3) rc = embed_fwd_pool_only(a, s);
   else if (a->parts != 2) rc = embed_fwd_layer1_heads(&a, &g1, 1, s, a->rows_staged ? 2 : 0);
   if (rc || a->parts == 1) return rc;
-  return launch_gemm(L_NT, g2, s, PS_EMBED_L2_FWD);
-}
-
-int lirec_embed_fwd2(const lirec_embed_fwd_args* a, const lirec_embed_fwd_args* b, lirec_stream_t stream) {
+  GemmGroup* gs[1] = {&g2};
+  const bool st = attach_fwd_sink(gs, 1, sink);
+  rc = launch_gemm(L_NT, g2, s, PS_EMBED_L2_FWD);
+  if (!rc && st) *staged = 1;
+  return rc;
+}
+
+int lirec_embed_fwd(const lirec_embed_fwd_args* a, lirec_stream_t stream) { return embed_fwd_impl(a, stream, nullptr, nullptr); }
+
+int lirec_embed_fwd_ws(const lirec_embed_fwd_args* a, void* ws, int64_t ws_bytes, int32_t gate_n, int32_t gate_K, int32_t gate_N,
+                       int32_t* staged, lirec_stream_t stream) {
+  const GateSink k = {ws, ws_bytes, gate_n, gate_K, gate_N};
+  if (gate_sink_args_bad(&k, staged)) return LIREC_EINVAL;
+  *staged = 0;
+  return embed_fwd_impl(a, stream, &k, staged);
+}
+
+static int embed_fwd2_impl(const lirec_embed_fwd_args* a, const lirec_embed_fwd_args* b, lirec_stream_t stream, const GateSink* sink,
+                           int32_t* staged) {
   GemmGroup g1[2], a2, b2, m2;
   int rc = embed_fwd_build(a, g1[0], a2);
   if (rc) return rc;
@@ -1198,9 +1251,27 @@
   if (a->parts == 3) { rc = embed_fwd_pool_only(a, s); if (!rc) rc = embed_fwd_pool_only(b, s); }
   else if (a->parts != 2) rc = embed_fwd_layer1_heads(hs, g1, 2, s, a->rows_staged ? 2 : 0);
   if (rc || a->parts == 1) return rc;
-  if (merge_groups(a2, b2, m2)) return launch_gemm(L_NT, m2, s, PS_EMBED_L2_FWD);
-  rc = launch_gemm(L_NT, a2, s, PS_EMBED_L2_FWD);
-  return rc ? rc : launch_gemm(L_NT, b2, s, PS_EMBED_L2_FWD);
+  GemmGroup* gs[2] = {&a2, &b2};
+  const bool st = attach_fwd_sink(gs, 2, sink);
+  if (merge_groups(a2, b2, m2)) rc = launch_gemm(L_NT, m2, s, PS_EMBED_L2_FWD);
+  else {
+    rc = launch_gemm(L_NT, a2, s, PS_EMBED_L2_FWD);
+    if (!rc) rc = launch_gemm(L_NT, b2, s, PS_EMBED_L2_FWD);
+  }
+  if (!rc && st) *staged = 1;
+  return rc;
+}
+
+int lirec_embed_fwd2(const lirec_embed_fwd_args* a, const lirec_embed_fwd_args* b, lirec_stream_t stream) {
+  return embed_fwd2_impl(a, b, stream, nullptr, nullptr);
+}
+
+int lirec_embed_fwd2_ws(const lirec_embed_fwd_args* a, const lirec_embed_fwd_args* b, void* ws, int64_t ws_bytes, int32_t gate_n,
+                        int32_t gate_K, int32_t gate_N, int32_t* staged, lirec_stream_t stream) {
+  const GateSink k = {ws, ws_bytes, gate_n, gate_K, gate_N};
+  if (gate_sink_args_bad(&k, staged)) return LIREC_EINVAL;
+  *staged = 0;
+  return embed_fwd2_impl(a, b, stream, &k, staged);
 }
 
 int lirec_embed_l1_indexed(const lirec_embed_fwd_args* const* heads, int32_t nh, const lirec_pieces* pc,
@@ -1813,7 +1884,6 @@
          (reinterpret_cast<uintptr_t>(ws) & 255) == 0 && n >= 32 && (n & 31) == 0 &&
          (K & 255) == 0 && (N & 255) == 0 && ldee == K && ws_bytes >= lirec_gate_ws_bytes(n, K, N);
 }
-struct GateWs { unsigned char* wq; unsigned char* eq; unsigned char* zq; unsigned char* wqT; unsigned char* eqT; unsigned char* zqT; };
 static GateWs gate_ws(void* ws, int n, int K, int N) {
   const long n32 = (n + 31) / 32 * 32;
   GateWs w;
@@ -1893,14 +1963,20 @@
 int lirec_gate_fwd_ws(const float* EE, int64_t ldee, const float* Wg, const float* bg, int32_t n, int32_t K,
                       int32_t N, float* G, int64_t ldg, const lirec_dropout* drop, void* ws, int64_t ws_bytes,
                       int32_t weights_staged, lirec_stream_t stream) {
+  return lirec_gate_fwd_ws2(EE, ldee, Wg, bg, n, K, N, G, ldg, drop, ws, ws_bytes, weights_staged, 0, stream);
+}
+
+int lirec_gate_fwd_ws2(const float* EE, int64_t ldee, const float* Wg, const float* bg, int32_t n, int32_t K,
+                       int32_t N, float* G, int64_t ldg, const lirec_dropout* drop, void* ws, int64_t ws_bytes,
+                       int32_t weights_staged, int32_t rows_staged, lirec_stream_t stream) {
   if (!EE || !Wg || !G || n < 0 || K < 1 || N < 1) return LIREC_EINVAL;
   if (!gate_q32_ok(n, K, N, ldee, ws, ws_bytes) || ((reinterpret_cast<uintptr_t>(EE) | reinterpret_cast<uintptr_t>(Wg)) & 15) != 0)
-    return weights_staged ? LIREC_EINVAL : lirec_gate_fwd(EE, ldee, Wg, bg, n, K, N, G, ldg, drop, stream);
+    return (weights_staged || rows_staged) ? LIREC_EINVAL : lirec_gate_fwd(EE, ldee, Wg, bg, n, K, N, G, ldg, drop, stream);
   hipStream_t s = (hipStream_t)stream;
   const GateWs w = gate_ws(ws, n, K, N);
   SplitDual q;
   memset(&q, 0, sizeof(q));
-  if ((!weights_staged && !dual_add(q, Wg, w.wq, w.wqT, N, K)) || !dual_add(q, EE, w.eq, w.eqT, n, K)) return LIREC_EINVAL;
+  if ((!weights_staged && !dual_add(q, Wg, w.wq, w.wqT, N, K)) || (!rows_staged && !dual_add(q, EE, w.eq, w.eqT, n, K))) return LIREC_EINVAL;
   int rc = launch_gate_stage(q, s);
   if (rc) return rc;
   GemmGroup g;
@@ -2032,9 +2108,11 @@
   return lirec_linear_fwd_group(&v, 1, stream);
 }
 
-int lirec_linear_bwd_group(const lirec_linear_bwd_args* v, int32_t count, lirec_stream_t stream) {
+static int linear_bwd_group_impl(const lirec_linear_bwd_args* v, int32_t count, lirec_stream_t stream, int stage_head, const GateSink* sink,
+                                 int32_t* staged) {
   if (!v || count < 1 || count > LIREC_MAX_PROB) return LIREC_EINVAL;
   hipStream_t s = (hipStream_t)stream;
+  bool st = false;
   if ((g_ablate & 131072) && v[0].parts != 2) lirec::launch(spin_kernel, dim3(1), dim3(64), 0, s, 200000LL);
   GemmGroup gw, gd;
   gw.nprob = 0; gd.nprob = 0;
@@ -2057,6 +2135,11 @@
     if (a.mode == 1) {
       p.epi = EPI_RELU_BWD; p.aux = a.act; p.ldaux = a.ldact;
       p.drop_scale = (pd > 0.f) ? (float)(1.0 / (1.0 - (double)pd)) : 1.f;
+      if (i == stage_head && a.n == sink->n && a.K == sink->N && a.ldda == sink->N && gate_sink_ok(sink)) {
+        const GateWs w = gate_ws(sink->ws, sink->n, sink->K, sink->N);
+        p.sq = w.zq; p.sqT = w.zqT; p.s_rbn = a.n >> 5; p.s_cbn = a.K >> 5; p.s_cb0 = 0;
+        st = true;
+      }
     } else if (a.mode == 2) {
       p.epi = EPI_TANH_BWD; p.aux = a.act; p.ldaux = a.ldact;
       set_dropout(p, &a.drop, a.drop.site2, 0);
@@ -2067,7 +2150,21 @@
   }
   int rc = launch_gemm(L_TN, gw, s, PS_LINEAR_DW);
   if (rc || gd.nprob == 0) return rc;
-  return launch_gemm(L_NN, gd, s, PS_LINEAR_DA);
+  rc = launch_gemm(L_NN, gd, s, PS_LINEAR_DA);
+  if (!rc && st) *staged = 1;
+  return rc;
+}
+
+int lirec_linear_bwd_group(const lirec_linear_bwd_args* v, int32_t count, lirec_stream_t stream) {
+  return linear_bwd_group_impl(v, count, stream, -1, nullptr, nullptr);
+}
+
+int lirec_linear_bwd_group_ws(const lirec_linear_bwd_args* v, int32_t count, int32_t stage_head, void* ws, int64_t ws_bytes,
+                              int32_t gate_n, int32_t gate_K, int32_t gate_N, int32_t* staged, lirec_stream_t stream) {
+  const GateSink k = {ws, ws_bytes, gate_n, gate_K, gate_N};
+  if (gate_sink_args_bad(&k, staged) || stage_head < 0 || stage_head >= count) return LIREC_EINVAL;
+  *staged = 0;
+  return linear_bwd_group_impl(v, count, stream, stage_head, &k, staged);
 }
 
 int lirec_linear_bwd(const float* dY, int64_t lddy, const float* A, int64_t lda, const float* W,
diff --git a/lirec_amd/model.py b/lirec_amd/model.py
--- a/lirec_amd/model.py
+++ b/lirec_amd/model.py
@@ -406,6 +406,7 @@
             lane0 = self._wgrad_lane()
             if lane0 is not None:
                 deferred_join = (ops.current_stream_handle(), C.c_void_p(lane0[0].cuda_stream))
+        sink = (st['gate_ws'], n, ldee, Wg.shape[0]) if has_g and st.get('gate_ws') is not None else None
         st['pieces'] = pieces if pq is None else None
         st['pieces_gather'] = pq if (pq is not None and isinstance(pieces['clip'], ops.Q32Block)) else None
         if pq is None and pieces is not None and isinstance(pieces['clip'], ops.Q32Block):
@@ -418,31 +419,33 @@
                 ops.stream_wait(*w_side)
             elif deferred_join is not None:
                 ops.stream_wait(*deferred_join)
-            ops.embed_fwd2(ops.with_parts(args_i, 3), ops.with_parts(args_c, 3))
+            ee_staged = ops.embed_fwd2(ops.with_parts(args_i, 3), ops.with_parts(args_c, 3), gate=sink)
             if has_g:
                 ops.gate_fwd(EE, ldee, Wg, bg, n, ldee, N, G, N, self._dropout(SITE_GATE), ws=st['gate_ws'],
-                             weights_staged=w_side is not None)
+                             weights_staged=w_side is not None, rows_staged=ee_staged)
         else:
             def layers(parts):
                 if has_i and has_c:
-                    ops.embed_fwd2(ops.with_parts(args_i, parts), ops.with_parts(args_c, parts)) if parts else ops.embed_fwd2(args_i, args_c)
+                    return ops.embed_fwd2(ops.with_parts(args_i, parts) if parts else args_i,
+                                          ops.with_parts(args_c, parts) if parts else args_c, gate=sink)
                 elif has_i:
-                    ops.embed_fwd(args=ops.with_parts(args_i, parts) if parts else args_i)
+                    return ops.embed_fwd(args=ops.with_parts(args_i, parts) if parts else args_i, gate=sink)
                 elif has_c:
-                    ops.embed_fwd(args=ops.with_parts(args_c, parts) if parts else args_c)
+                    return ops.embed_fwd(args=ops.with_parts(args_c, parts) if parts else args_c)
+                return False
             if has_g and w_side is not None:
                 layers(1)
                 ops.stream_wait(*w_side)
-                layers(2)
+                ee_staged = layers(2)
             elif deferred_join is not None:
                 layers(1)
                 ops.stream_wait(*deferred_join)
-                layers(2)
+                ee_staged = layers(2)
             else:
-                layers(0)
+                ee_staged = layers(0)
             if has_g:
                 ops.gate_fwd(EE, ldee, Wg, bg, n, ldee, N, G, N, self._dropout(SITE_GATE), ws=st['gate_ws'],
-                             weights_staged=w_side is not None)
+                             weights_staged=w_side is not None, rows_staged=ee_staged)
         heads = []
         if has_i:
             Wo, bo = self._W('out_ints')
@@ -561,12 +564,15 @@
                               self._g('out_ints.weight'), self._g('out_ints.bias'), _ptr(dEE, Wc), ldee,
                               2, _ptr(Tn, Wc), ldee, 0, drop(0, SITE_E_INTS)))
         one_fork = bool(heads) and lane is not None and has_i and has_g
+        sink = dict(gate=(st['gate_ws'], n, ldee, st['G'].shape[1]), stage_head=len(heads) - 1) \
+            if has_i and has_g and st.get('gate_ws') is not None else {}
+        dzg_staged = False
         if heads and lane is not None:
             if not one_fork:
                 on_side(lambda: ops.linear_bwd_group(heads, parts=1))
-            ops.linear_bwd_group(heads, parts=2)
+            dzg_staged = ops.linear_bwd_group(heads, parts=2, **sink)
         elif heads:
-            ops.linear_bwd_group(heads)
+            dzg_staged = ops.linear_bwd_group(heads, **sink)
         if has_i and has_g:
             G = st['G']
             N = G.shape[1]
@@ -575,8 +581,8 @@
                                               self._g('gates_ints.fc_out.weight'), self._g('gates_ints.fc_out.bias'),
                                               dEE, ldee, has_c, drop(0), SITE_E_CTX, SITE_E_INTS, parts=parts,
                                               ws=st.get('gate_ws'), rows_staged=staged)
-            staged = False
-            if st.get('gate_ws') is not None and lane is not None:
+            staged = dzg_staged
+            if st.get('gate_ws') is not None and lane is not None and not staged:
                 gate(4)
                 staged = True
             if one_fork:
diff --git a/lirec_amd/ops.py b/lirec_amd/ops.py
--- a/lirec_amd/ops.py
+++ b/lirec_amd/ops.py
@@ -284,13 +284,29 @@
     return a
 
 
+def _gate_sink(gate):
+    ws, n, K, N = gate
+    return _p(ws) if ws is not None else None, (ws.numel() * ws.element_size() if ws is not None else 0), int(n), int(K), int(N), C.c_int32(0)
+
+
 def embed_fwd(*args, **kw):
+    gate = kw.pop('gate', None)
     a = kw['args'] if 'args' in kw else embed_fwd_args(*args, **kw)
+    if gate is not None:
+        ws, nb, n, K, N, staged = _gate_sink(gate)
+        check(lib().lirec_embed_fwd_ws(C.byref(a), ws, nb, n, K, N, C.byref(staged), _stream()), 'lirec_embed_fwd_ws')
+        return bool(staged.value)
     check(lib().lirec_embed_fwd(C.byref(a), _stream()), 'lirec_embed_fwd')
-
-
-def embed_fwd2(a, b):
+    return False
+
+
+def embed_fwd2(a, b, gate=None):
+    if gate is not None:
+        ws, nb, n, K, N, staged = _gate_sink(gate)
+        check(lib().lirec_embed_fwd2_ws(C.byref(a), C.byref(b), ws, nb, n, K, N, C.byref(staged), _stream()), 'lirec_embed_fwd2_ws')
+        return bool(staged.value)
     check(lib().lirec_embed_fwd2(C.byref(a), C.byref(b), _stream()), 'lirec_embed_fwd2')
+    return False
 
 
 def embed_bwd_args(X, ldx, sel, rows, J, segs: Segments, W2, H1, dZ2, lddz2, dW1, db1, dW2, db2, workspace, drop,
@@ -471,10 +487,11 @@
     return True
 
 
-def gate_fwd(EE, ldee, Wg, bg, n, K, N, G, ldg, drop, ws=None, weights_staged=False):
+def gate_fwd(EE, ldee, Wg, bg, n, K, N, G, ldg, drop, ws=None, weights_staged=False, rows_staged=False):
     if ws is not None:
-        check(lib().lirec_gate_fwd_ws(_p(EE), ldee, _p(Wg), _p(bg), n, K, N, _p(G), ldg, C.byref(drop), _p(ws),
-                                      ws.numel() * ws.element_size(), int(weights_staged), _stream()), 'lirec_gate_fwd_ws')
+        check(lib().lirec_gate_fwd_ws2(_p(EE), ldee, _p(Wg), _p(bg), n, K, N, _p(G), ldg, C.byref(drop), _p(ws),
+                                       ws.numel() * ws.element_size(), int(weights_staged), int(rows_staged), _stream()),
+              'lirec_gate_fwd_ws2')
         return
     check(lib().lirec_gate_fwd(_p(EE), ldee, _p(Wg), _p(bg), n, K, N, _p(G), ldg, C.byref(drop), _stream()),
           'lirec_gate_fwd')
@@ -503,14 +520,20 @@
     check(lib().lirec_linear_fwd_group(arr, len(items), _stream()), 'lirec_linear_fwd_group')
 
 
-def linear_bwd_group(items, parts=0):
+def linear_bwd_group(items, parts=0, gate=None, stage_head=None):
     arr = (LinearBwdArgs * len(items))()
     for v, (dY, lddy, A, lda, W, n, K, N, dW, db, dA, ldda, mode, act, ldact, accumulate, drop) in zip(arr, items):
         v.dY, v.lddy, v.A, v.lda, v.W = _p(dY), lddy, A, lda, _p(W)
         v.dW, v.db, v.dA, v.ldda, v.act, v.ldact = _p(dW), _p(db), dA, ldda, act, ldact
         v.n, v.K, v.N, v.mode, v.accumulate, v.parts = n, K, N, mode, int(accumulate), int(parts)
         v.drop = drop
+    if gate is not None and stage_head is not None:
+        ws, nb, n, K, N, staged = _gate_sink(gate)
+        check(lib().lirec_linear_bwd_group_ws(arr, len(items), int(stage_head), ws, nb, n, K, N, C.byref(staged), _stream()),
+              'lirec_linear_bwd_group_ws')
+        return bool(staged.value)
     check(lib().lirec_linear_bwd_group(arr, len(items), _stream()), 'lirec_linear_bwd_group')
+    return False
 
 
 def linear_bwd(dY, lddy, A, lda, W, n, K, N, dW, db, dA, ldda, mode, act, ldact, accumulate, drop):
```

Result: no change. 79420, median of 6 (+0.7%).
